# JCBrouwer/maua-style

Measured on AMD Instinct MI355X. Metric: optimizer iterations/sec at 1024x1024 VGG-19, higher is better.
Workload: dtype f32 (fp16x3 split-precision MFMA, fp32 accumulate)

## Files before the change

### include/maua_hip.h

```cpp
#ifndef MAUA_HIP_H
#define MAUA_HIP_H

#include <stddef.h>
#include <stdint.h>

#ifdef __cplusplus
extern "C" {
#endif

typedef void* maua_stream_t;

#define MAUA_OK 0
#define MAUA_E_INVAL (-1)
#define MAUA_E_UNSUPPORTED (-2)
#define MAUA_E_WORKSPACE (-3)

int maua_abi_version(void);
const char* maua_last_error(void);


int maua_conv_pack_filters(const float* w_oihw, float* wf, float* wb, int cout, int cin, int kh, int kw,
                           maua_stream_t stream);

size_t maua_conv_workspace_bytes(int n, int cin, int h, int w, int cout, int kh, int kw, int stride, int pad);
// ... 3 lines not shown

int maua_conv2d_bwd_data(const float* gy, const float* out_mask, const float* wb, const float* w_oihw,
                         const float* in_relu_mask, float* gx, int n, int cin, int h, int w, int cout, int kh, int kw,
                         int stride, int pad, int accumulate, void* workspace, size_t workspace_bytes, maua_stream_t stream);

size_t maua_conv_x6_bank_bytes(int cout_produced, int cin_consumed);
int maua_conv_pack_filters_x6(const float* w_oihw, void* bank_fwd, void* bank_bwd, int cout, int cin, maua_stream_t stream);
size_t maua_conv_x6_workspace_bytes(int n, int cin, int h, int w, int cout, int pad);
int maua_conv3x3_x6(const float* x, const void* bank, const float* bias, const float* out_relu_mask, float* y, int n,
                    int cin, int h, int w, int cout, int pad, int relu, int accumulate, void* workspace,
                    size_t workspace_bytes, maua_stream_t stream);

int maua_conv_image_supported(int n, int cin, int h, int w, int cout, int pad);
size_t maua_conv_image_bank_bytes(int cout, int cin);
int maua_conv_pack_filters_image(const float* w_oihw, const float* bias, void* bank, int cout, int cin, maua_stream_t stream);
int maua_conv3x3_image(const float* x, const void* bank, float* y, int n, int cin, int h, int w, int cout, int pad, int relu,
                       maua_stream_t stream);
int maua_conv_image_gram_slabs(int h, int w, int pad);
int maua_conv3x3_image_gram(const float* x, const void* bank, float* y, float* gram_slabs, int cin, int h, int w, int pad, maua_stream_t stream);

size_t maua_conv_x3_bank_bytes(int cout_produced, int cin_consumed);
int maua_conv_pack_filters_x3(const float* w_oihw, void* bank_fwd, void* bank_bwd, int cout, int cin, float w_scale,
                              maua_stream_t stream);
size_t maua_conv_x3_workspace_bytes(int n, int cin, int h, int w, int cout, int pad);
int maua_conv3x3_x3(const float* x, const void* bank, float w_scale, const float* bias, const float* out_relu_mask, float* y,
                    int n, int cin, int h, int w, int cout, int pad, int relu, int accumulate, void* workspace,
                    size_t workspace_bytes, maua_stream_t stream);

size_t maua_conv_x3w_bank_bytes(int cout_produced, int cin_consumed);
int maua_conv_pack_filters_x3w(const float* w_oihw, void* bank_fwd, void* bank_bwd, int cout, int cin, float w_scale,
                               maua_stream_t stream);
int maua_conv_x3w_supported(int cin, int h, int w, int pad);
size_t maua_conv_x3w_workspace_bytes(int n, int cin, int h, int w, int cout, int pad);
int maua_conv3x3_x3w(const float* x, const void* bank, float w_scale, const float* bias, const float* out_relu_mask, float* y,
                     int n, int cin, int h, int w, int cout, int pad, int relu, int accumulate, void* workspace,
                     size_t workspace_bytes, maua_stream_t stream);

int maua_conv_x3w_split(int n, int cin, int h, int w, int cout, int pad);
int maua_conv3x3_x3w_relu_pool(const float* x, const void* bank, float w_scale, const float* bias, float* pooled,
                               unsigned char* codes, int n, int cin, int h, int w, int cout, int pad, void* workspace,
                               size_t workspace_bytes, maua_stream_t stream);

size_t maua_conv_x3w_dmat_bank_bytes(int c);
int maua_conv_pack_dmat_x3w(const float* dmat, int c, void* bank, float* inv_scale_out, maua_stream_t stream);
int maua_conv_pack_dmat_x3w_batch(int count, const float* const* dmats, const int* cs, void* const* banks, float* const* inv_scales_out,
                                  maua_stream_t stream);
int maua_conv3x3_x3w_gram(const float* x, const void* bank, float w_scale, const float* feature_map, const void* dmat_bank,
                          const float* dmat_inv_scale, float* y, int n, int cin, int h, int w, int cout, int pad, int accumulate,
                          void* workspace, size_t workspace_bytes, maua_stream_t stream);

int maua_conv3x3_x3w_unpool(const float* pooled_x, const unsigned char* codes, int honour_relu_bit, const void* bank, float w_scale,
                            const float* out_relu_mask, const void* dmat_bank, const float* dmat_inv_scale, float* y, int n, int cin,
                            int h, int w, int cout, int pad, void* workspace, size_t workspace_bytes, maua_stream_t stream);

size_t maua_conv_x3q_bank_bytes(int cout_produced, int cin_consumed);
int maua_conv_pack_filters_x3q(const float* w_oihw, void* bank_fwd, void* bank_bwd, int cout, int cin, float w_scale,
                               maua_stream_t stream);
int maua_conv_x3q_supported(int cin, int h, int w, int pad);
size_t maua_conv_x3q_workspace_bytes(int n, int cin, int h, int w, int cout, int pad);
int maua_conv_x3q_split(int n, int cin, int h, int w, int cout, int pad);
int maua_conv_x3q_preferred(int n, int cin, int h, int w, int cout, int pad);
int maua_conv3x3_x3q(const float* x, const void* bank, float w_scale, const float* bias, const float* out_relu_mask, float* y,
                     int n, int cin, int h, int w, int cout, int pad, int relu, int accumulate, void* workspace,
                     size_t workspace_bytes, maua_stream_t stream);
int maua_conv3x3_x3q_relu_pool(const float* x, const void* bank, float w_scale, const float* bias, float* pooled, unsigned char* codes,
                               int n, int cin, int h, int w, int cout, int pad, void* workspace, size_t workspace_bytes,
                               maua_stream_t stream);
int maua_conv3x3_x3q_unpool(const float* pooled_x, const unsigned char* codes, int honour_relu_bit, const void* bank, float w_scale,
                            const float* out_relu_mask, float* y, int n, int cin, int h, int w, int cout, int pad, void* workspace,
                            size_t workspace_bytes, maua_stream_t stream);

int maua_conv_x3p_supported(int cin, int h, int w, int cout, int pad);
int maua_conv_x3p_split(int n, int cin, int h, int w, int cout, int pad);
size_t maua_conv_x3p_workspace_bytes(int n, int cin, int h, int w, int cout, int pad);
int maua_conv_x3p_preferred(int n, int cin, int h, int w, int cout, int pad);
int maua_conv_x3p_set_max_groups(int groups);
int maua_conv3x3_x3p(const float* x, const unsigned char* in_codes, int honour_relu_bit, const void* bank, float w_scale, const float* bias,
                     const float* out_relu_mask, const void* dmat_bank, const float* dmat_inv_scale, float* y, unsigned char* pool_codes,
                     int n, int cin, int h, int w, int cout, int pad, int relu, void* workspace, size_t workspace_bytes, maua_stream_t stream);

size_t maua_conv_kxk_x3_bank_bytes(int cout_produced, int cin_consumed, int ks);
int maua_conv_pack_filters_kxk_x3(const float* w_oihw, void* bank_fwd, void* bank_bwd, int cout, int cin, int ks, float w_scale,
                                  maua_stream_t stream);
size_t maua_conv_kxk_x3_workspace_bytes(int n, int cin, int h, int w, int cout, int ks, int pad);
int maua_conv_kxk_x3(const float* x, const void* bank, float w_scale, const float* bias, const float* out_relu_mask, float* y,
                     int n, int cin, int h, int w, int cout, int ks, int pad, int relu, int accumulate, void* workspace,
                     size_t workspace_bytes, maua_stream_t stream);

size_t maua_conv1x1_x3_workspace_bytes(int n, int cin, int64_t hw, int cout);
int maua_conv1x1_x3(const float* x, const float* x_channel_shift, const float* w_rowmajor, const float* bias,
                    const float* out_relu_mask, float* y, int n, int cin, int64_t hw, int cout, int relu, int accumulate,
                    void* workspace, size_t workspace_bytes, maua_stream_t stream);

int maua_relu_fwd(float* x_inplace, int64_t count, maua_stream_t stream);
int maua_relu_bwd(const float* gy, const float* y, float* gx, int64_t count, maua_stream_t stream);

int maua_pool_out_size(int in, int k, int stride, int ceil_mode);
int maua_pool2d_fwd(const float* x, float* y, int n, int c, int h, int w, int k, int stride, int ceil_mode, int mode,
                    maua_stream_t stream);
int maua_pool2d_bwd(const float* gy, const float* x, float* gx, int n, int c, int h, int w, int k, int stride,
                    int ceil_mode, int mode, int relu_mask_by_x, maua_stream_t stream);

int maua_pool2x2_codes_supported(int n, int c, int h, int w);
int maua_pool2x2_fwd_codes(const float* x, float* y, unsigned char* codes, int n, int c, int h, int w, maua_stream_t stream);
int maua_pool2x2_bwd_codes(const float* gy, const unsigned char* codes, float* gx, int n, int c, int h, int w, int relu_mask,
                           maua_stream_t stream);

size_t maua_gram_workspace_bytes(int c, int64_t hw);
int maua_gram_block(int c, int64_t hw);
int maua_gram_fwd(const float* f, float* gram, float* row_mean_out, int c, int64_t hw, float scale, int center,
                  void* workspace, size_t workspace_bytes, maua_stream_t stream);

size_t maua_reduce_workspace_bytes(int64_t count);
int maua_mse_fwd_bwd(const float* x, const float* target, float* grad, int64_t count, float loss_scale, float grad_scale,
                     int accumulate, int mask_grad_by_x, float* loss_out, void* workspace, size_t workspace_bytes,
                     maua_stream_t stream);
int maua_mse_weighted_fwd_bwd(const float* x, const float* weights, const float* target, float* grad, int64_t planes,
                              int64_t plane, int weight_planes, float loss_scale, float grad_scale, int accumulate,
                              float* loss_out, void* workspace, size_t workspace_bytes, maua_stream_t stream);

int maua_gram_bwd(const float* d_sym, const float* f, const float* row_mean, const float* relu_mask, float* gf, int c,
                  int64_t hw, int accumulate, void* workspace, size_t workspace_bytes, maua_stream_t stream);

int maua_tv_fwd_bwd(const float* x, float* grad, int n, int c, int h, int w, float strength, int accumulate,
                    float* loss_out, void* workspace, size_t workspace_bytes, maua_stream_t stream);

size_t maua_loss_ledger_bytes(int frames, int slots);
int maua_mse_fwd_bwd_ledger(const float* x, const float* target, float* grad, int64_t count, float loss_scale, float grad_scale,
                            int accumulate, int mask_grad_by_x, double* ledger, int slot, maua_stream_t stream);
int maua_tv_fwd_bwd_ledger(const float* x, float* grad, int n, int c, int h, int w, float strength, int accumulate,
                           double* ledger, int slot, maua_stream_t stream);
int maua_gram_mse_ledger_supported(int c);
int maua_gram_fwd_mse_ledger(const float* f, float* gram, float* row_mean_out, int c, int64_t hw, float scale, int center,
                             const float* target, float* dmat, float loss_scale, float grad_scale, double* ledger, int slot,
                             void* workspace, size_t workspace_bytes, maua_stream_t stream);
int maua_gram_partial(const float* f, float* row_mean_out, int c, int64_t hw, int center, void* workspace, size_t workspace_bytes,
                      maua_stream_t stream);
int maua_gram_partial_batch(int count, const float* const* fs, float* const* means, const int* cs, const int64_t* hws,
                            void* const* workspaces, const size_t* workspace_bytes, const int* slab_counts, maua_stream_t stream);
int maua_gram_row_means(const float* f, float* row_mean_out, int c, int64_t hw, void* workspace, size_t workspace_bytes, maua_stream_t stream);
int maua_gram_finish_mse_batch(int count, const void* const* workspaces, float* const* grams, const float* const* targets,
                               float* const* dmats, const int* cs, const int64_t* hws, const float* scales, const float* loss_scales,
                               const float* grad_scales, double* const* ledgers, const int* slots, const int* slab_counts,
                               maua_stream_t stream);
int maua_loss_ledger_sum(double* ledger, int frames, int slots, float* losses, float* totals, maua_stream_t stream);
int maua_loss_ledger_sum_f64(double* ledger, int frames, int slots, float* losses, float* totals, double* losses_f64,
                             maua_stream_t stream);

int maua_fill(float* x, int64_t count, float value, maua_stream_t stream);
size_t maua_conv_few_mfma_bank_bytes(void);
int maua_conv_pack_filters_few_mfma(const float* w_oihw, void* bank, int cout, int cin, maua_stream_t stream);
int maua_conv_few_mfma_supported(int n, int cin, int h, int w, int cout, int pad);
int maua_conv3x3_few_mfma(const float* gy, const void* bank, float* gx, int n, int cin, int h, int w, int cout, int tile, maua_stream_t stream);

int maua_space_to_depth(const float* in, float* out, int n, int c_in, int r, int h, int w, int qh, int qw, maua_stream_t stream);
int maua_depth_to_space(const float* in, float* out, int n, int c_out, int r, int qh, int qw, int h, int w, int accumulate, maua_stream_t stream);
int maua_axpy(float* y, const float* x, float alpha, int64_t count, maua_stream_t stream);
int maua_sum_small(const float* in, int count, float* out, maua_stream_t stream);

int maua_adam_step(float* x, const float* grad, float* exp_avg, float* exp_avg_sq, int64_t count, int step, float lr,
                   float beta1, float beta2, float eps, maua_stream_t stream);

size_t maua_channel_stats_workspace_bytes(int h, int w);
int maua_channel_stats(const float* x_bchw, const float* noise_bwhc, float noise_amp, int frames, int slot, int h, int w,
                       double* stats9, void* workspace, size_t workspace_bytes, maua_stream_t stream);
int maua_color_match_solve(const double* stats_target, int frames, int64_t pixels_target, const double* stats_source,
                           int64_t pixels_source, float eps, float* coef16, maua_stream_t stream);
int maua_color_match_apply(const float* x_bchw, const float* noise_bwhc, float noise_amp, const float* coef16, const float* all_coef,
                           int n_coef, float weight, int accumulate, int frames, int slot, int h, int w, float* out_bchw,
                           maua_stream_t stream);
int maua_resize_bilinear(const float* x, float* y, int planes, int h, int w, int oh, int ow, float scale_h, float scale_w,
                         maua_stream_t stream);
int maua_deprocess_u8(const float* x_bgr_chw, unsigned char* out_rgb_hwc, int h, int w, float mean_b, float mean_g, float mean_r,
                      maua_stream_t stream);

int maua_set_tuning(const char* name, double value);
double maua_get_tuning(const char* name, double dflt);

void maua_set_split_batch_hint(int frames);
int maua_get_split_batch_hint(void);

int maua_conv_arm_workspace(void* workspace, void* counters, size_t counter_bytes, int zero, maua_stream_t stream);

size_t maua_lbfgs_state_bytes(int64_t count, int history);
int maua_lbfgs_init(void* state, size_t state_bytes, int64_t count, int history, maua_stream_t stream);
int maua_lbfgs_iterate(void* state, float* x, const float* grad, const float* loss, int64_t count, int history, float lr,
                       float tolerance_change, float tolerance_grad, maua_stream_t stream);
int maua_lbfgs_status(const void* state, int64_t count, int history, float* out5, maua_stream_t stream);

int maua_flow_levels(int h, int w, int max_levels);
int maua_flow_grey_u8(const uint8_t* rgb, float* out, int h, int w, maua_stream_t stream);
int maua_flow_pyr_down(const float* in, float* out, int h, int w, maua_stream_t stream);
int maua_flow_warp_prep(const float* i0, const float* i1, const float* u, float* fields, int h, int w, maua_stream_t stream);
int maua_flow_tvl1_step(const float* fields, const float* state_in, float* state_out, int h, int w, maua_stream_t stream);
int maua_flow_tvl1_blocked(const float* fields, const float* state_in, float* state_out, int h, int w, int k, maua_stream_t stream);
int maua_flow_median5(const float* in, float* out, int h, int w, int planes, maua_stream_t stream);
int maua_flow_upsample(const float* in, int ch, int cw, float* out, int h, int w, int planes, float scale, maua_stream_t stream);
size_t maua_flow_consistency_workspace_bytes(int h, int w);
int maua_flow_consistency(const float* flow1, const float* flow2, uint8_t* out, int h, int w, void* workspace, size_t workspace_bytes,
                          maua_stream_t stream);
size_t maua_flow_tvl1_workspace_bytes(int h, int w, int levels);
int maua_flow_tvl1(const uint8_t* rgb1, const uint8_t* rgb2, float* flow, int h, int w, int levels, int warps, int iters, int block_k,
                   void* workspace, size_t workspace_bytes, maua_stream_t stream);

int maua_nca_supported(int n, int chn, int hidden, int h, int w);
int64_t maua_nca_param_count(int chn, int hidden);
int maua_nca_step(const float* x, float* out, const float* params, int n, int chn, int hidden, int h, int w, float rate,
                  const float* rate_map, const float* mask, uint64_t seed, int64_t step, maua_stream_t stream);
size_t maua_nca_bwd_workspace_bytes(int n, int chn, int hidden, int h, int w);
int maua_nca_step_bwd(const float* x, const float* g, float* dx, const float* params, int n, int chn, int hidden, int h, int w,
                      float rate, const float* rate_map, const float* mask, uint64_t seed, int64_t step, int first, void* workspace,
                      size_t workspace_bytes, maua_stream_t stream);
int maua_nca_grad_finish(float* grad, int n, int chn, int hidden, int h, int w, const void* workspace, size_t workspace_bytes,
                         int normalize, maua_stream_t stream);

#ifdef __cplusplus
}
#endif
#endif
```

### maua-style_amd/csrc/conv_api.hip

```cpp
#include <cstdlib>
#include <cstring>

#include "common.hpp"

using namespace maua;

namespace maua {
static thread_local int g_split_batch_hint = 1;
int split_batch_hint() { return g_split_batch_hint; }
static thread_local const void* g_armed_ws = nullptr;
static thread_local unsigned* g_armed_counters = nullptr;
unsigned* armed_counters(const void* workspace) { return workspace && workspace == g_armed_ws ? g_armed_counters : nullptr; }
}

namespace maua {
static const char* const g_tuning_names[] = {"conv_few_out", "few_out_ks4_below", "x3w_ks", "x3w_stagger", "x3q_ks", "x3q_min_fill", "x3q_min_chunks",
                                             "x3p_ks", "x3p_groups", "x3p_min_fill", "x3p_min_items", "x6_persist", "gram_x3", "gram_bwd_x3",
                                             "gram_t128", "gram_t128_min_hw", "p1_order", "lbfgs_vec", "lbfgs_tri", "finish_in_launch_max_ks", "x3p_order", "cot_inner"};
constexpr int kTunings = sizeof(g_tuning_names) / sizeof(g_tuning_names[0]);
static double g_tuning_values[kTunings];
static bool g_tuning_set[kTunings];
static int tuning_index(const char* name) {
    for (int i = 0; i < kTunings; ++i)
        if (name && strcmp(name, g_tuning_names[i]) == 0) return i;
    return -1;
}
double tuning(const char* name, double dflt) {
    const int i = tuning_index(name);
    return i >= 0 && g_tuning_set[i] ? g_tuning_values[i] : dflt;
}
}

static inline bool mfma_geometry(int kh, int kw, int stride) {
    return stride == 1 && kh == kw && (kh == 1 || kh == 3 || kh == 5);
}
static int conv_route(const ConvArgs& a, int ks, int n, hipStream_t stream) {
    const bool few_out = tuning("conv_few_out", 1) != 0;
    if (ks == 3 && a.Cout <= 4 && a.Cin >= 16 && few_out) return conv3x3_few_out(a, n, stream);
    return conv_mfma_dispatch(a, ks, n, stream);
}

extern "C" {

int maua_set_tuning(const char* name, double value) {
    const int i = maua::tuning_index(name);
    MAUA_REQUIRE(i >= 0, MAUA_E_INVAL, "set_tuning: unknown constant %s", name ? name : "(null)");
    maua::g_tuning_values[i] = value;
    maua::g_tuning_set[i] = true;
    return MAUA_OK;
}
double maua_get_tuning(const char* name, double dflt) { return maua::tuning(name, dflt); }

int maua_conv_arm_workspace(void* workspace, void* counters, size_t counter_bytes, int zero, maua_stream_t stream) {
    if (!workspace || !counters) {
        maua::g_armed_ws = nullptr;
        maua::g_armed_counters = nullptr;
        return MAUA_OK;
    }
    MAUA_REQUIRE(counter_bytes >= (size_t)maua::ARRIVE_COUNTERS * 4 && ((size_t)counters & 15) == 0, MAUA_E_INVAL,
                 "conv_arm_workspace: needs %d bytes of 16-byte aligned counters", maua::ARRIVE_COUNTERS * 4);
    const hipError_t rc = zero ? hipMemsetAsync(counters, 0, (size_t)maua::ARRIVE_COUNTERS * 4, (hipStream_t)stream) : hipSuccess;
    if (rc != hipSuccess) {
        set_error("conv_arm_workspace: hipMemsetAsync: %s", hipGetErrorString(rc));
        return (int)rc;
    }
    maua::g_armed_ws = workspace;
    maua::g_armed_counters = (unsigned*)counters;
    return MAUA_OK;
}

void maua_set_split_batch_hint(int frames) { maua::g_split_batch_hint = frames > 0 ? frames : 1; }
int maua_get_split_batch_hint(void) { return maua::g_split_batch_hint; }

size_t maua_conv_workspace_bytes(int n, int cin, int h, int w, int cout, int kh, int kw, int stride, int pad) {
    if (!conv_dims_ok(n, cin, h, w, cout, pad) || kh <= 0 || kw <= 0 || kh > 64 || kw > 64 || stride <= 0 || stride > 64) return 0;
    if (!mfma_geometry(kh, kw, stride) || h + 2 * pad < kh || w + 2 * pad < kw) return 0;
    ConvArgs a{};
    a.Cin = cin;
    a.Cout = cout;
    a.OH = h + 2 * pad - kh + 1;
    a.OW = w + 2 * pad - kw + 1;
    if (kh == 3 && cout <= 4 && cin >= 16) return 0;
    const int ks = conv_mfma2_choose_split(a, kh, n);
    return ks > 1 ? (size_t)n * ks * cout * a.OH * a.OW * sizeof(float) : 0;
}

int maua_conv2d_fwd(const float* x, const float* in_mask, const float* wf, const float* bias, float* y, int n, int cin,
                    int h, int w, int cout, int kh, int kw, int stride, int pad, int relu, int accumulate, void* workspace,
                    size_t workspace_bytes, maua_stream_t stream) {
    MAUA_REQUIRE(x && wf && y, MAUA_E_INVAL, "conv2d_fwd: null pointer");
    MAUA_REQUIRE(conv_dims_ok(n, cin, h, w, cout, pad) && kh > 0 && kw > 0 && kh <= 64 && kw <= 64 && stride > 0 && stride <= 64, MAUA_E_INVAL,
                 "conv2d_fwd: bad dims n=%d cin=%d cout=%d h=%d w=%d k=%dx%d s=%d p=%d", n, cin, cout, h, w, kh, kw, stride,
                 pad);
    const int oh = (h + 2 * pad - kh) / stride + 1, ow = (w + 2 * pad - kw) / stride + 1;
    MAUA_REQUIRE(h + 2 * pad >= kh && w + 2 * pad >= kw, MAUA_E_UNSUPPORTED, "conv2d_fwd: input %dx%d smaller than filter", h,
                 w);
    MAUA_REQUIRE((int64_t)h * w < (1ll << 31) && (int64_t)oh * ow < (1ll << 31), MAUA_E_UNSUPPORTED,
                 "conv2d_fwd: plane too large");
    if (mfma_geometry(kh, kw, stride)) {
        ConvArgs a{};
        a.x = x;
        a.mask = in_mask;
        a.w = wf;
        a.bias = bias;
        a.y = y;
        a.Cin = cin;
        a.H = h;
        a.W = w;
        a.Cout = cout;
        a.OH = oh;
        a.OW = ow;
        a.pad = pad;
        a.relu = relu;
        a.accumulate = accumulate;
        a.ws = (workspace && workspace_bytes >= maua_conv_workspace_bytes(n, cin, h, w, cout, kh, kw, stride, pad))
                   ? (float*)workspace : nullptr;
        return conv_route(a, kh, n, (hipStream_t)stream);
    }
    return conv_direct_fwd(x, in_mask, wf, bias, y, n, cin, h, w, cout, oh, ow, kh, kw, stride, pad, relu, accumulate,
                           (hipStream_t)stream);
}

int maua_conv2d_bwd_data(const float* gy, const float* out_mask, const float* wb, const float* w_oihw,
                         const float* in_relu_mask, float* gx, int n, int cin, int h, int w, int cout, int kh, int kw,
                         int stride, int pad, int accumulate, void* workspace, size_t workspace_bytes, maua_stream_t stream) {
    MAUA_REQUIRE(gy && gx && (wb || w_oihw), MAUA_E_INVAL, "conv2d_bwd_data: null pointer");
    MAUA_REQUIRE(conv_dims_ok(n, cin, h, w, cout, pad) && kh > 0 && kw > 0 && kh <= 64 && kw <= 64 && stride > 0 && stride <= 64, MAUA_E_INVAL,
                 "conv2d_bwd_data: bad dims");
    const int oh = (h + 2 * pad - kh) / stride + 1, ow = (w + 2 * pad - kw) / stride + 1;
    MAUA_REQUIRE(h + 2 * pad >= kh && w + 2 * pad >= kw, MAUA_E_UNSUPPORTED, "conv2d_bwd_data: input smaller than filter");
    if (mfma_geometry(kh, kw, stride) && wb) {
        ConvArgs a{};
        a.x = gy;
        a.mask = out_mask;
        a.w = wb;
        a.bias = nullptr;
        a.omask = in_relu_mask;
        a.y = gx;
        a.Cin = cout;
        a.H = oh;
        a.W = ow;
        a.Cout = cin;
        a.OH = h;
        a.OW = w;
        a.pad = kh - 1 - pad;
        a.relu = 0;
        a.accumulate = accumulate;
        MAUA_REQUIRE(a.pad >= 0, MAUA_E_UNSUPPORTED, "conv2d_bwd_data: pad %d > k-1", pad);
        a.ws = (workspace && workspace_bytes >= maua_conv_workspace_bytes(n, cout, oh, ow, cin, kh, kw, 1, a.pad))
                   ? (float*)workspace : nullptr;
        return conv_route(a, kh, n, (hipStream_t)stream);
    }
    MAUA_REQUIRE(w_oihw, MAUA_E_INVAL, "conv2d_bwd_data: the direct path needs the OIHW weights");
    return conv_direct_bwd(gy, out_mask, w_oihw, in_relu_mask, gx, n, cin, h, w, cout, oh, ow, kh, kw, stride, pad, accumulate,
                           (hipStream_t)stream);
}

}
```

### maua-style_amd/csrc/conv_few_mfma.hip

```cpp
#include <hip/hip_runtime.h>

#include "common.hpp"

namespace maua {

typedef __attribute__((ext_vector_type(8))) __bf16 fm_bf16x8;
typedef __attribute__((ext_vector_type(16))) float fm_f32x16;
typedef __attribute__((ext_vector_type(4))) unsigned int fm_u32x4;
typedef float fm_f32x2 __attribute__((ext_vector_type(2)));
typedef __bf16 fm_bf16x2 __attribute__((ext_vector_type(2)));

__device__ __forceinline__ unsigned short fm_bf16_bits(float x) { return __builtin_bit_cast(unsigned short, (__bf16)x); }
__device__ __forceinline__ float fm_bf16_value(unsigned short u) { return __builtin_bit_cast(float, (unsigned)u << 16); }
__device__ __forceinline__ unsigned fm_cvt_pk(float a, float b) {
    const fm_f32x2 v = {a, b};
    return __builtin_bit_cast(unsigned, __builtin_convertvector(v, fm_bf16x2));
}

constexpr int FM_K = 64;
constexpr int FM_STEPS = FM_K / 16;
constexpr int FM_TC = 64, FM_OC = 62;
constexpr int FM_BANK_BYTES = FM_STEPS * 3 * 64 * 16;

__global__ void pack_few_mfma_kernel(const float* __restrict__ w, unsigned short* __restrict__ bank, int co) {
    const int total = FM_STEPS * 64 * 8;
    for (int e = blockIdx.x * blockDim.x + threadIdx.x; e < total; e += gridDim.x * blockDim.x) {
        const int i = e % 8, lane = (e / 8) % 64, step = e / 512;
        const int m = lane & 31, k = 16 * step + 8 * (lane >> 5) + i;
        float v = 0.f;
        if (m < 9 * co) {
            const int tap = m / co, c = m - tap * co;
            v = w[((int64_t)k * co + c) * 9 + tap];
        }
        const unsigned short h = fm_bf16_bits(v);
        const float r1 = v - fm_bf16_value(h);
        const unsigned short md = fm_bf16_bits(r1);
        const unsigned short l = fm_bf16_bits(r1 - fm_bf16_value(md));
        const unsigned short parts[3] = {h, md, l};
        for (int part = 0; part < 3; ++part) bank[(((int64_t)step * 3 + part) * 64 + lane) * 8 + i] = parts[part];
    }
}

struct FewMfmaArgs {
    const float* gy;
    const unsigned char* bank;
    float* gx;
    int H, W, co;
    int tiles_x, tiles, per_xcd;
};

template <int ROWS>
__global__ void __launch_bounds__(256, 2) conv_few_mfma_kernel(FewMfmaArgs p) {
    extern __shared__ float T[];
    constexpr int TR = ROWS + 2, TPL = TR * FM_TC, NBLK = TR * 2;
    const int tid = threadIdx.x, lane = tid & 63, wave = tid >> 6, nl = lane & 31, kg = lane >> 5;
    const int tile = (int)(blockIdx.x & 7) * p.per_xcd + (int)(blockIdx.x >> 3);
    if (tile >= p.tiles) return;
    const int ty = tile / p.tiles_x;
    const int x0 = (tile - ty * p.tiles_x) * FM_OC, y0 = ty * ROWS, img = blockIdx.z;
    const int64_t plane = (int64_t)p.H * p.W;
    fm_bf16x8 a[FM_STEPS][3];
#pragma unroll
    for (int step = 0; step < FM_STEPS; ++step)
#pragma unroll
        for (int part = 0; part < 3; ++part)
            a[step][part] = *reinterpret_cast<const fm_bf16x8*>(p.bank + (((step * 3 + part) * 64) + lane) * 16);
    const __amdgpu_buffer_rsrc_t rs = __builtin_amdgcn_make_buffer_rsrc(const_cast<float*>(p.gy) + (int64_t)img * FM_K * plane, 0,
                                                                        (unsigned)(FM_K * plane * 4), 0x00020000);
    auto request = [&](float (&v)[FM_STEPS][8], int b) {
        const int tr = b >> 1, Y = y0 - 1 + tr, X = x0 - 1 + 32 * (b & 1) + nl;
        const bool ok = Y >= 0 && Y < p.H && X >= 0 && X < p.W;
        const unsigned voff = ok ? (unsigned)(((int64_t)kg * 8 * plane + (int64_t)Y * p.W + X) * 4) : 0x80000000u;
#pragma unroll
        for (int step = 0; step < FM_STEPS; ++step)
#pragma unroll
            for (int i = 0; i < 8; ++i)
                v[step][i] = __builtin_bit_cast(float, __builtin_amdgcn_raw_buffer_load_b32(rs, voff, (unsigned)((16 * step + i) * plane * 4), 0));
    };
    float v[FM_STEPS][8], vn[FM_STEPS][8];
    if (wave < NBLK) request(v, wave);
    for (int b = wave; b < NBLK; b += 4) {
        if (b + 4 < NBLK) request(vn, b + 4);
        fm_f32x16 acc;
#pragma unroll
        for (int r = 0; r < 16; ++r) acc[r] = 0.f;
#pragma unroll
        for (int step = 0; step < FM_STEPS; ++step) {
            fm_u32x4 bp[3];
#pragma unroll
            for (int q = 0; q < 4; ++q) {
                const float u0 = v[step][2 * q], u1 = v[step][2 * q + 1];
                const unsigned h = fm_cvt_pk(u0, u1);
                const float r0 = u0 - __builtin_bit_cast(float, h << 16), r1 = u1 - __builtin_bit_cast(float, h & 0xffff0000u);
                const unsigned m = fm_cvt_pk(r0, r1);
                const unsigned l = fm_cvt_pk(r0 - __builtin_bit_cast(float, m << 16), r1 - __builtin_bit_cast(float, m & 0xffff0000u));
                bp[0][q] = h;
                bp[1][q] = m;
                bp[2][q] = l;
            }
            const fm_bf16x8 b0v = __builtin_bit_cast(fm_bf16x8, bp[0]), b1v = __builtin_bit_cast(fm_bf16x8, bp[1]),
                            b2v = __builtin_bit_cast(fm_bf16x8, bp[2]);
            acc = __builtin_amdgcn_mfma_f32_32x32x16_bf16(a[step][2], b0v, acc, 0, 0, 0);
            acc = __builtin_amdgcn_mfma_f32_32x32x16_bf16(a[step][1], b1v, acc, 0, 0, 0);
            acc = __builtin_amdgcn_mfma_f32_32x32x16_bf16(a[step][0], b2v, acc, 0, 0, 0);
            acc = __builtin_amdgcn_mfma_f32_32x32x16_bf16(a[step][1], b0v, acc, 0, 0, 0);
            acc = __builtin_amdgcn_mfma_f32_32x32x16_bf16(a[step][0], b1v, acc, 0, 0, 0);
            acc = __builtin_amdgcn_mfma_f32_32x32x16_bf16(a[step][0], b0v, acc, 0, 0, 0);
        }
        float* dst = T + (b >> 1) * FM_TC + 32 * (b & 1) + nl;
#pragma unroll
        for (int r = 0; r < 16; ++r) {
            const int m = (r & 3) + 8 * (r >> 2) + 4 * kg;
            if (m < 9 * p.co) dst[m * TPL] = acc[r];
        }
#pragma unroll
        for (int step = 0; step < FM_STEPS; ++step)
#pragma unroll
            for (int i = 0; i < 8; ++i) v[step][i] = vn[step][i];
    }
    __syncthreads();
    const int co = p.co;
    for (int idx = tid; idx < ROWS * FM_OC; idx += 256) {
        const int i = idx / FM_OC, j = idx - i * FM_OC;
        const int Y = y0 + i, X = x0 + j;
        if (Y >= p.H || X >= p.W) continue;
        const float* t0 = T + (i + 2) * FM_TC + j + 2;
        for (int c = 0; c < co; ++c) {
            float s = 0.f;
#pragma unroll
            for (int ky = 0; ky < 3; ++ky)
#pragma unroll
                for (int kx = 0; kx < 3; ++kx) s += t0[((ky * 3 + kx) * co + c) * TPL - ky * FM_TC - kx];
            p.gx[((int64_t)img * co + c) * plane + (int64_t)Y * p.W + X] = s;
        }
    }
}

}

using namespace maua;

extern "C" {

size_t maua_conv_few_mfma_bank_bytes(void) { return FM_BANK_BYTES; }

int maua_conv_pack_filters_few_mfma(const float* w_oihw, void* bank, int cout, int cin, maua_stream_t stream) {
    MAUA_REQUIRE(w_oihw && bank, MAUA_E_INVAL, "conv_pack_filters_few_mfma: null pointer");
    MAUA_REQUIRE(cout == FM_K && cin >= 1 && cin <= 3, MAUA_E_UNSUPPORTED, "conv_pack_filters_few_mfma: a 3x3 layer with %d filters over 1-3 channels (got %d over %d)", FM_K, cout, cin);
    hipLaunchKernelGGL(pack_few_mfma_kernel, dim3(8), dim3(256), 0, (hipStream_t)stream, w_oihw, (unsigned short*)bank, cin);
    return check_launch("pack_few_mfma_kernel");
}

int maua_conv_few_mfma_supported(int n, int cin, int h, int w, int cout, int pad) {
    return conv_dims_ok(n, cin, h, w, cout, pad) && cout == FM_K && cin >= 1 && cin <= 3 && pad == 1 && n <= 65535 && (int64_t)FM_K * h * w * 4 < (1ll << 31) &&
           (h + 3) / 4 <= 65535;
}

int maua_conv3x3_few_mfma(const float* gy, const void* bank, float* gx, int n, int cin, int h, int w, int cout, int tile, maua_stream_t stream) {
    MAUA_REQUIRE(gy && bank && gx, MAUA_E_INVAL, "conv3x3_few_mfma: null pointer");
    MAUA_REQUIRE(maua_conv_few_mfma_supported(n, cin, h, w, cout, 1), MAUA_E_UNSUPPORTED, "conv3x3_few_mfma: unsupported geometry");
    MAUA_REQUIRE(tile >= 0 && tile <= 3, MAUA_E_INVAL, "conv3x3_few_mfma: tile code 0 - 3");
    if (tile == 0) tile = (int64_t)h * w < 1000000 ? 1 : 2;
    FewMfmaArgs p{gy, (const unsigned char*)bank, gx, h, w, cin, 0, 0, 0};
    static unsigned long long attr[4] = {0, 0, 0, 0};
    const int rows = tile == 1 ? 4 : tile == 2 ? 8 : 14;
    const int lds = 27 * (rows + 2) * FM_TC * 4;
    p.tiles_x = (w + FM_OC - 1) / FM_OC;
    p.tiles = p.tiles_x * ((h + rows - 1) / rows);
    p.per_xcd = (p.tiles + 7) / 8;
    const dim3 grid((unsigned)(8 * p.per_xcd), 1, (unsigned)n);
    if (rows == 4) {
        (void)opt_in_dynamic_lds(reinterpret_cast<const void*>(conv_few_mfma_kernel<4>), lds, &attr[1]);
        hipLaunchKernelGGL(conv_few_mfma_kernel<4>, grid, dim3(256), lds, (hipStream_t)stream, p);
    } else if (rows == 8) {
        (void)opt_in_dynamic_lds(reinterpret_cast<const void*>(conv_few_mfma_kernel<8>), lds, &attr[2]);
        hipLaunchKernelGGL(conv_few_mfma_kernel<8>, grid, dim3(256), lds, (hipStream_t)stream, p);
    } else {
        (void)opt_in_dynamic_lds(reinterpret_cast<const void*>(conv_few_mfma_kernel<14>), lds, &attr[3]);
        hipLaunchKernelGGL(conv_few_mfma_kernel<14>, grid, dim3(256), lds, (hipStream_t)stream, p);
    }
    return check_launch("conv_few_mfma_kernel");
}

}
```

### maua-style_amd/csrc/conv_img.hip

```cpp
#include <hip/hip_runtime.h>

#include "common.hpp"

namespace maua {

typedef __attribute__((ext_vector_type(8))) __bf16 ci_bf16x8;
typedef __attribute__((ext_vector_type(16))) float ci_f32x16;
typedef __attribute__((ext_vector_type(4))) unsigned int ci_u32x4;
typedef float ci_f32x2 __attribute__((ext_vector_type(2)));
typedef __bf16 ci_bf16x2 __attribute__((ext_vector_type(2)));

__device__ __forceinline__ unsigned short ci_bf16_bits(float x) { return __builtin_bit_cast(unsigned short, (__bf16)x); }
__device__ __forceinline__ float ci_bf16_value(unsigned short u) { return __builtin_bit_cast(float, (unsigned)u << 16); }
__device__ __forceinline__ unsigned ci_cvt_pk(float a, float b) {
    const ci_f32x2 v = {a, b};
    return __builtin_bit_cast(unsigned, __builtin_convertvector(v, ci_bf16x2));
}

constexpr int CI_KPAD = 32;
#ifndef CI_OCC
#define CI_OCC 2
#endif
constexpr int CI_TILE_BYTES = 2 * 2 * 3 * 64 * 16;

__global__ void pack_image_kernel(const float* __restrict__ w, const float* __restrict__ bias, unsigned short* __restrict__ bank, int cout,
                                  int cin) {
    const int ntile = (cout + 63) / 64;
    const int64_t total = (int64_t)ntile * 2 * 2 * 64 * 8;
    for (int64_t e = (int64_t)blockIdx.x * blockDim.x + threadIdx.x; e < total; e += (int64_t)gridDim.x * blockDim.x) {
        int64_t r = e;
        const int i = (int)(r % 8);
        r /= 8;
        const int lane = (int)(r % 64);
        r /= 64;
        const int step = (int)(r % 2);
        r /= 2;
        const int blk = (int)(r % 2);
        const int tile = (int)(r / 2);
        const int co = tile * 64 + blk * 32 + (lane & 31), k = 16 * step + 8 * (lane >> 5) + i;
        float v = 0.f;
        if (co < cout && k < 9 * cin) v = w[(int64_t)co * cin * 9 + k];
        if (co < cout && k == 9 * cin && bias) v = bias[co];
        const unsigned short h = ci_bf16_bits(v);
        const float r1 = v - ci_bf16_value(h);
        const unsigned short m = ci_bf16_bits(r1);
        const unsigned short l = ci_bf16_bits(r1 - ci_bf16_value(m));
        const unsigned short parts[3] = {h, m, l};
        for (int part = 0; part < 3; ++part)
            bank[(((((int64_t)tile * 2 + blk) * 2 + step) * 3 + part) * 64 + lane) * 8 + i] = parts[part];
    }
}

struct ImgArgs {
    const float* x;
    const unsigned char* bank;
    float* y;
    float* gram_slabs;
    int n, cin, H, W, cout, OH, OW, pad, relu;
    int blocks_x;
    int64_t blocks;
};

template <bool GRAM>
__global__ void __launch_bounds__(256, CI_OCC) conv_image_kernel(ImgArgs p) {
    const int lane = threadIdx.x & 63;
    const int nl = lane & 31, kg = lane >> 5;
    const int tile = blockIdx.y;
    ci_bf16x8 a[2][2][3];
    {
        const unsigned char* src = p.bank + (int64_t)tile * CI_TILE_BYTES + lane * 16;
#pragma unroll
        for (int blk = 0; blk < 2; ++blk)
#pragma unroll
            for (int step = 0; step < 2; ++step)
#pragma unroll
                for (int part = 0; part < 3; ++part)
                    a[blk][step][part] = *reinterpret_cast<const ci_bf16x8*>(src + (((blk * 2 + step) * 3 + part) * 64) * 16);
    }
    const int64_t plane = (int64_t)p.H * p.W;
    const int kmax = 9 * p.cin;
    int rel[2][8];
    unsigned ones = 0;
#pragma unroll
    for (int step = 0; step < 2; ++step)
#pragma unroll
        for (int i = 0; i < 8; ++i) {
            int k = 16 * step + 8 * kg + i;
            if (k == kmax) ones |= 1u << (8 * step + i);
            k = k < kmax ? k : 0;
            const int ci = k / 9, ky = (k - 9 * ci) / 3, kx = k - 9 * ci - 3 * ky;
            rel[step][i] = (int)(ci * plane) + (ky - p.pad) * p.W + (kx - p.pad);
        }
    const int64_t out_plane = (int64_t)p.OH * p.OW;
    const int nw = (int)gridDim.x * 4;
    const int wid = __builtin_amdgcn_readfirstlane((int)blockIdx.x * 4 + (int)(threadIdx.x >> 6));
    const int per = (int)((p.blocks + nw - 1) / nw);
    const int b0 = wid * per, b1 = (int)(p.blocks < (int64_t)b0 + per ? p.blocks : (int64_t)b0 + per);
    ci_f32x16 gsum[3];
    if constexpr (GRAM) {
#pragma unroll
        for (int q = 0; q < 3; ++q)
#pragma unroll
            for (int r = 0; r < 16; ++r) gsum[q][r] = 0.f;
    }
    if (!GRAM && b0 >= b1) return;
    int bx = b0 < b1 ? b0 % p.blocks_x : 0, oy = b0 < b1 ? (b0 / p.blocks_x) % p.OH : 0, img = b0 < b1 ? (b0 / p.blocks_x) / p.OH : 0;
    auto gather = [&](float (&v)[2][8], int gi, int gy, int gb) {
        const int ox = gb * 32 + nl;
        const float* __restrict__ xin = p.x + (int64_t)gi * p.cin * plane;
        const int centre = gy * p.W + ox;
        const bool interior = gy - p.pad >= 0 && gy - p.pad + 2 < p.H && gb * 32 - p.pad >= 0 && gb * 32 + 31 - p.pad + 2 < p.W;
        if (interior) {
#pragma unroll
            for (int step = 0; step < 2; ++step)
#pragma unroll
                for (int i = 0; i < 8; ++i) v[step][i] = xin[centre + rel[step][i]];
        } else {
#pragma unroll
            for (int step = 0; step < 2; ++step)
#pragma unroll
                for (int i = 0; i < 8; ++i) {
                    int k = 16 * step + 8 * kg + i;
                    k = k < kmax ? k : 0;
                    const int t9 = k % 9;
                    const int iy = gy + t9 / 3 - p.pad, ix = ox + t9 % 3 - p.pad;
                    const bool ok = iy >= 0 && iy < p.H && ix >= 0 && ix < p.W;
                    v[step][i] = ok ? xin[centre + rel[step][i]] : 0.f;
                }
        }
    };
    float v[2][8], vn[2][8];
    if (b0 < b1) gather(v, img, oy, bx);
    for (int b = b0; b < b1; ++b) {
        bx = __builtin_amdgcn_readfirstlane(bx);
        oy = __builtin_amdgcn_readfirstlane(oy);
        img = __builtin_amdgcn_readfirstlane(img);
        int nbx = bx + 1, noy = oy, nimg = img;
        if (nbx == p.blocks_x) {
            nbx = 0;
            if (++noy == p.OH) {
                noy = 0;
                ++nimg;
            }
        }
        if (b + 1 < b1) gather(vn, nimg, noy, nbx);
#pragma unroll
        for (int step = 0; step < 2; ++step)
#pragma unroll
            for (int i = 0; i < 8; ++i) v[step][i] = (ones >> (8 * step + i)) & 1u ? 1.f : v[step][i];
        ci_u32x4 bp[2][3];
#pragma unroll
        for (int step = 0; step < 2; ++step)
#pragma unroll
            for (int q = 0; q < 4; ++q) {
                const float x0 = v[step][2 * q], x1 = v[step][2 * q + 1];
                const unsigned h = ci_cvt_pk(x0, x1);
                const float r0 = x0 - __builtin_bit_cast(float, h << 16), r1 = x1 - __builtin_bit_cast(float, h & 0xffff0000u);
                const unsigned m = ci_cvt_pk(r0, r1);
                const unsigned l = ci_cvt_pk(r0 - __builtin_bit_cast(float, m << 16), r1 - __builtin_bit_cast(float, m & 0xffff0000u));
                bp[step][0][q] = h;
                bp[step][1][q] = m;
                bp[step][2][q] = l;
            }
        ci_f32x16 acc[2];
#pragma unroll
        for (int blk = 0; blk < 2; ++blk)
#pragma unroll
            for (int r = 0; r < 16; ++r) acc[blk][r] = 0.f;
#pragma unroll
        for (int step = 0; step < 2; ++step) {
            const ci_bf16x8 b0v = __builtin_bit_cast(ci_bf16x8, bp[step][0]), b1v = __builtin_bit_cast(ci_bf16x8, bp[step][1]),
                            b2v = __builtin_bit_cast(ci_bf16x8, bp[step][2]);
#define CI_PAIR(AP, BV)                                                                                         \
    acc[0] = __builtin_amdgcn_mfma_f32_32x32x16_bf16(a[0][step][AP], BV, acc[0], 0, 0, 0);                       \
    acc[1] = __builtin_amdgcn_mfma_f32_32x32x16_bf16(a[1][step][AP], BV, acc[1], 0, 0, 0);
            CI_PAIR(2, b0v) CI_PAIR(1, b1v) CI_PAIR(0, b2v) CI_PAIR(1, b0v) CI_PAIR(0, b1v) CI_PAIR(0, b0v)
#undef CI_PAIR
        }
        const int ox = bx * 32 + nl;
        const int tile_ch = min(64, p.cout - tile * 64);
        const __amdgpu_buffer_rsrc_t rs = __builtin_amdgcn_make_buffer_rsrc(p.y + ((int64_t)img * p.cout + tile * 64) * out_plane, 0,
                                                                            (unsigned)(tile_ch * out_plane * 4), 0x00020000);
        const unsigned voff = ox < p.OW ? (unsigned)((4 * kg * out_plane + (int64_t)oy * p.OW + ox) * 4) : 0x80000000u;
#pragma unroll
        for (int blk = 0; blk < 2; ++blk)
#pragma unroll
            for (int r = 0; r < 16; ++r) {
                const int cr = blk * 32 + (r & 3) + 8 * (r >> 2);
                float o = acc[blk][r];
                if (p.relu) o = o > 0.f ? o : 0.f;
                __builtin_amdgcn_raw_buffer_store_b32(__builtin_bit_cast(unsigned, o), rs, voff, (int)(cr * out_plane * 4), 0);
            }
        if constexpr (GRAM) {
            ci_f32x16 xt[2];
#pragma unroll
            for (int blk = 0; blk < 2; ++blk)
#pragma unroll
                for (int r = 0; r < 16; ++r) xt[blk][r] = 0.f;
#pragma unroll
            for (int step = 0; step < 2; ++step) {
                const ci_bf16x8 b0v = __builtin_bit_cast(ci_bf16x8, bp[step][0]), b1v = __builtin_bit_cast(ci_bf16x8, bp[step][1]),
                                b2v = __builtin_bit_cast(ci_bf16x8, bp[step][2]);
#define CI_PAIR_T(AP, BV)                                                                                       \
    xt[0] = __builtin_amdgcn_mfma_f32_32x32x16_bf16(BV, a[0][step][AP], xt[0], 0, 0, 0);                         \
    xt[1] = __builtin_amdgcn_mfma_f32_32x32x16_bf16(BV, a[1][step][AP], xt[1], 0, 0, 0);
                CI_PAIR_T(2, b0v) CI_PAIR_T(1, b1v) CI_PAIR_T(0, b2v) CI_PAIR_T(1, b0v) CI_PAIR_T(0, b1v) CI_PAIR_T(0, b0v)
#undef CI_PAIR_T
            }
            ci_u32x4 fr[2][2][3];
            const int px0 = bx * 32 + 4 * kg;
#pragma unroll
            for (int blk = 0; blk < 2; ++blk)
#pragma unroll
                for (int sK = 0; sK < 2; ++sK)
#pragma unroll
                    for (int q = 0; q < 4; ++q) {
                        const int r0i = 8 * sK + 2 * q, r1i = r0i + 1;
                        float x0 = xt[blk][r0i], x1 = xt[blk][r1i];
                        x0 = (x0 > 0.f && px0 + (r0i & 3) + 8 * (r0i >> 2) < p.OW) ? x0 : 0.f;
                        x1 = (x1 > 0.f && px0 + (r1i & 3) + 8 * (r1i >> 2) < p.OW) ? x1 : 0.f;
                        const unsigned h = ci_cvt_pk(x0, x1);
                        const float e0 = x0 - __builtin_bit_cast(float, h << 16), e1 = x1 - __builtin_bit_cast(float, h & 0xffff0000u);
                        const unsigned m = ci_cvt_pk(e0, e1);
                        const unsigned l = ci_cvt_pk(e0 - __builtin_bit_cast(float, m << 16), e1 - __builtin_bit_cast(float, m & 0xffff0000u));
                        fr[blk][sK][0][q] = h;
                        fr[blk][sK][1][q] = m;
                        fr[blk][sK][2][q] = l;
                    }
#pragma unroll
            for (int sK = 0; sK < 2; ++sK) {
#define CI_G(PA, PB)                                                                                                                        \
    gsum[0] = __builtin_amdgcn_mfma_f32_32x32x16_bf16(__builtin_bit_cast(ci_bf16x8, fr[0][sK][PA]), __builtin_bit_cast(ci_bf16x8, fr[0][sK][PB]), gsum[0], 0, 0, 0); \
    gsum[1] = __builtin_amdgcn_mfma_f32_32x32x16_bf16(__builtin_bit_cast(ci_bf16x8, fr[0][sK][PA]), __builtin_bit_cast(ci_bf16x8, fr[1][sK][PB]), gsum[1], 0, 0, 0); \
    gsum[2] = __builtin_amdgcn_mfma_f32_32x32x16_bf16(__builtin_bit_cast(ci_bf16x8, fr[1][sK][PA]), __builtin_bit_cast(ci_bf16x8, fr[1][sK][PB]), gsum[2], 0, 0, 0);
                CI_G(2, 0) CI_G(1, 1) CI_G(0, 2) CI_G(1, 0) CI_G(0, 1) CI_G(0, 0)
#undef CI_G
            }
        }
#pragma unroll
        for (int step = 0; step < 2; ++step)
#pragma unroll
            for (int i = 0; i < 8; ++i) v[step][i] = vn[step][i];
        bx = nbx;
        oy = noy;
        img = nimg;
    }
    if constexpr (GRAM) {
        __shared__ float red[3][3][16][64];
        const int wave = threadIdx.x >> 6;
        if (wave > 0) {
#pragma unroll
            for (int q = 0; q < 3; ++q)
#pragma unroll
                for (int r = 0; r < 16; ++r) red[wave - 1][q][r][lane] = gsum[q][r];
        }
        __syncthreads();
        if (wave > 0) return;
        float* __restrict__ slab = p.gram_slabs + (int64_t)blockIdx.x * 64 * 64;
#pragma unroll
        for (int q = 0; q < 3; ++q) {
            const int bi = q == 2 ? 1 : 0, bj = q == 0 ? 0 : 1;
#pragma unroll
            for (int r = 0; r < 16; ++r) {
                float g = gsum[q][r];
#pragma unroll
                for (int w = 0; w < 3; ++w) g += red[w][q][r][lane];
                slab[(bi * 32 + (r & 3) + 8 * (r >> 2) + 4 * kg) * 64 + bj * 32 + nl] = g;
            }
        }
    }
}

}

using namespace maua;

extern "C" {

size_t maua_conv_image_bank_bytes(int cout, int cin) {
    if (cout <= 0 || cin <= 0 || cin > 3 || cout > (1 << 16)) return 0;
    return (size_t)((cout + 63) / 64) * CI_TILE_BYTES;
}

int maua_conv_pack_filters_image(const float* w_oihw, const float* bias, void* bank, int cout, int cin, maua_stream_t stream) {
    MAUA_REQUIRE(w_oihw && bank && cout > 0 && cout <= (1 << 16) && cin > 0 && cin <= 3, MAUA_E_INVAL,
                 "conv_pack_filters_image: needs 1-3 input channels");
    hipLaunchKernelGGL(pack_image_kernel, dim3(32), dim3(256), 0, (hipStream_t)stream, w_oihw, bias, (unsigned short*)bank, cout, cin);
    return check_launch("pack_image_kernel");
}

static bool conv_image_fits(int64_t n, int64_t cin, int64_t h, int64_t w, int64_t pad) {
    const int64_t oh = h + 2 * pad - 2, ow = w + 2 * pad - 2;
    return cin * h * w < (1ll << 31) && n * oh * ((ow + 31) / 32) < (1ll << 31) && 64 * oh * ow < (1ll << 30);
}

static int conv_image_fill(ImgArgs& p, const float* x, const void* bank, float* y, int n, int cin, int h, int w, int cout, int pad, int relu) {
    MAUA_REQUIRE(x && bank && y, MAUA_E_INVAL, "conv3x3_image: null pointer");
    MAUA_REQUIRE(conv_dims_ok(n, cin, h, w, cout, pad) && pad <= 2 && cin <= 3, MAUA_E_INVAL, "conv3x3_image: bad dims (1-3 input channels)");
    MAUA_REQUIRE(h + 2 * pad >= 3 && w + 2 * pad >= 3, MAUA_E_UNSUPPORTED, "conv3x3_image: input smaller than the filter");
    MAUA_REQUIRE(conv_image_fits(n, cin, h, w, pad), MAUA_E_UNSUPPORTED, "conv3x3_image: plane too large (maua_conv_image_supported)");
    p.x = x;
    p.bank = (const unsigned char*)bank;
    p.y = y;
    p.n = n;
    p.cin = cin;
    p.H = h;
    p.W = w;
    p.cout = cout;
    p.OH = h + 2 * pad - 2;
    p.OW = w + 2 * pad - 2;
    p.pad = pad;
    p.relu = relu;
    p.blocks_x = (p.OW + 31) / 32;
    p.blocks = (int64_t)n * p.OH * p.blocks_x;
    return MAUA_OK;
}
static unsigned conv_image_grid(int64_t blocks) {
    const int64_t want = (blocks + 3) / 4;
    return (unsigned)(want < 256 * CI_OCC ? (want > 0 ? want : 1) : 256 * CI_OCC);
}

int maua_conv3x3_image(const float* x, const void* bank, float* y, int n, int cin, int h, int w, int cout, int pad, int relu,
                       maua_stream_t stream) {
    ImgArgs p{};
    const int rc = conv_image_fill(p, x, bank, y, n, cin, h, w, cout, pad, relu);
    if (rc) return rc;
    hipLaunchKernelGGL(conv_image_kernel<false>, dim3(conv_image_grid(p.blocks), (unsigned)((cout + 63) / 64)), dim3(256), 0, (hipStream_t)stream, p);
    return check_launch("conv_image_kernel");
}

int maua_conv_image_supported(int n, int cin, int h, int w, int cout, int pad) {
    return conv_dims_ok(n, cin, h, w, cout, pad) && pad <= 2 && cin <= 3 && h + 2 * pad >= 3 && w + 2 * pad >= 3 && conv_image_fits(n, cin, h, w, pad);
}

int maua_conv_image_gram_slabs(int h, int w, int pad) {
    if (h <= 0 || w <= 0 || pad < 0 || pad > 2 || h + 2 * pad < 3 || w + 2 * pad < 3 || !conv_image_fits(1, 3, h, w, pad)) return 0;
    const int64_t oh = h + 2 * pad - 2, ow = w + 2 * pad - 2;
    return (int)conv_image_grid(oh * ((ow + 31) / 32));
}

int maua_conv3x3_image_gram(const float* x, const void* bank, float* y, float* gram_slabs, int cin, int h, int w, int pad, maua_stream_t stream) {
    MAUA_REQUIRE(gram_slabs, MAUA_E_INVAL, "conv3x3_image_gram: null slabs");
    ImgArgs p{};
    const int rc = conv_image_fill(p, x, bank, y, 1, cin, h, w, 64, pad, 1);
    if (rc) return rc;
    p.gram_slabs = gram_slabs;
    hipLaunchKernelGGL(conv_image_kernel<true>, dim3(conv_image_grid(p.blocks), 1), dim3(256), 0, (hipStream_t)stream, p);
    return check_launch("conv_image_kernel");
}

}
```

### maua-style_amd/engine.py

```python
import contextlib
import os

import torch

import hip
import loss as loss_mod
import models as models_mod
import plan


class UnsupportedNet(RuntimeError):
    """The module sequence contains something the fused plan does not cover (callers fall back to running the
    modules one by one, which still executes on the GPU through the same kernels)."""


def _scale_grad_coeff(incoming, strength):
    g = float(incoming)
    return g / (abs(g) + 1e-8) * strength * strength


class _Step:
    __slots__ = ("kind", "mod", "relu", "src", "dst", "slot", "k", "stride", "pad", "ceil", "mode")

    def __init__(self, kind, mod=None):
# ... 123 lines not shown
                if len(users) == 1 and users[0].kind == "pool" and id(users[0]) in self.pool_codes and \
                        self._x6_ok(s, s.mod.out_channels) and models_mod.conv3x3_fwd_is_x3w(s.mod, *shapes[s.src][2:]) and \
                        s.mod.out_channels % 8 == 0 and (plan.on("fuse_pool_split") or models_mod.conv3x3_fwd_family(
                            s.mod, B, shapes[s.src][2], shapes[s.src][3])[1] == 1):
                    self.fused_pool[id(s)] = users[0]
        self.pooled_by_conv = {id(v) for v in self.fused_pool.values()}
        for s in self.steps:
            if id(s) in self.fused_pool:
                self.act[s.dst] = torch.empty(shapes[s.dst], device="meta")
        self.fused_unpool, self.pool_groups = {}, set()
        if self.x6_bwd:
            for s in self.steps:
                if s.kind != "conv" or not s.relu or s.k != 3 or s.stride != 1 or s.pad != 1:
                    continue
                users = [t for t in self.steps if t.src == s.dst and t is not s]
                if len(users) == 1 and users[0].kind == "pool" and id(users[0]) in self.pool_codes and \
                        self._x6_ok(s, s.mod.in_channels) and models_mod.conv3x3_bwd_is_x3w(s.mod, *shapes[s.dst][2:]):
                    self.pool_groups.add(id(s))
                    if plan.on("fuse_unpool"):
                        self.fused_unpool[id(s)] = users[0]
                        self.gbuf[s.dst] = torch.empty(shapes[s.dst], device="meta")
        self.unpooled_by_conv = {id(v) for v in self.fused_unpool.values()}
        self.fused_gram = {}
        max_c = plan.get_int("fuse_gram_max_c")
        if (B == 1 or self.independent) and self.x6_bwd and max_c > 0:
            relu_out = {s.dst for s in self.steps if s.kind == "conv" and s.relu}
            for s in self.steps:
                if s.kind != "conv" or s.k != 3 or s.stride != 1 or s.pad != 1 or s.src not in relu_out:
                    continue
                on_src = [t for t in self.steps if t.kind in ("style", "content") and t.src == s.src]
                c, h, w = shapes[s.src][1:]
                if len(on_src) == 1 and on_src[0].kind == "style" and not on_src[0].mod.use_covariance and c % 16 == 0 and \
                        c <= max_c and self._x6_ok(s, s.mod.in_channels) and models_mod.conv3x3_bwd_is_x3w(s.mod, *shapes[s.dst][2:]):
                    bank = hip.conv_x3w_dmat_bank(c, dev, B)
                    if bank is not None:
                        self.fused_gram[id(s)] = (on_src[0], bank[0], bank[1])
        self.fused_style = {id(v[0]): v for v in self.fused_gram.values()}
        self.image_gram = {}
        if B == 1 and self.batch_hint == 1 and self.ledger is not None and self.x6_fwd and plan.on("image_gram") and \
                plan.on("gram_x3") and models_mod._image_kernel_enabled():
            for s in self.steps:
                if s.kind != "conv" or not s.relu or s.k != 3 or s.stride != 1 or s.mod.in_channels > 3 or s.mod.out_channels != 64 or \
                        not self._x6_ok(s, 64):
                    continue
                on_dst = [t for t in self.steps if t.kind == "style" and t.src == s.dst]
                if len(on_dst) == 1 and not on_dst[0].mod.use_covariance and hip.gram_mse_ledger_supported(64):
                    h, w = shapes[s.src][2:]
                    slabs = hip.conv_image_gram_slabs(h, w, s.pad)
                    if 0 < slabs * 64 * 64 * 4 <= hip.gram_workspace_bytes(64, shapes[s.dst][2] * shapes[s.dst][3]):
                        self.image_gram[id(s)] = (on_dst[0], slabs)
        self.gram, self.dmat, self.mean = {}, {}, {}
        self.gram_d, self.dmat_d, self.mean_d = {}, {}, {}
        ws = hip.reduce_workspace_bytes(max(t.numel() for t in self.gbuf.values()))
        for s in self.steps:
            if s.kind == "style":
                c = shapes[s.src][1]
                hw = shapes[s.src][2] * shapes[s.src][3]
                self.gram[id(s)] = torch.empty(B, c, c, device=dev) if B > 1 else torch.empty(c, c, device=dev)
                self.dmat[id(s)] = torch.empty(B, c, c, device=dev) if B > 1 else torch.empty(c, c, device=dev)
                self.mean[id(s)] = (torch.empty(B, c, device=dev) if B > 1 else torch.empty(c, device=dev)) \
                    if s.mod.use_covariance else None
                ws = max(ws, hip.gram_workspace_bytes(c, hw), 4 * c + 256)
                if B > 1 and not self.independent:
                    self.gram_d[id(s)] = torch.empty(B * c, B * c, device=dev)
                    self.dmat_d[id(s)] = torch.empty(B * c, B * c, device=dev)
                    self.mean_d[id(s)] = torch.empty(B * c, device=dev) if s.mod.use_covariance else None
                    ws = max(ws, hip.gram_workspace_bytes(B * c, hw), 4 * B * c + 256)
        for s in self.steps:
            if s.kind == "conv" and s.stride == 1:
                n, cin, h, w = shapes[s.src]
                _, cout, oh, ow = shapes[s.dst]
                ws = max(ws, hip.conv_workspace_bytes(n, cin, h, w, cout, s.k, 1, s.pad),
                         hip.conv_workspace_bytes(n, cout, oh, ow, cin, s.k, 1, s.k - 1 - s.pad))
                if s.k == 5:
                    ws = max(ws, hip.conv_kxk_x3_workspace_bytes(n, cin, h, w, cout, 5, s.pad),
                             hip.conv_kxk_x3_workspace_bytes(n, cout, oh, ow, cin, 5, 4 - s.pad))
                if s.k == 1 and s.pad == 0:
                    ws = max(ws, hip.conv1x1_x3_workspace_bytes(n, cin, h * w, cout), hip.conv1x1_x3_workspace_bytes(n, cout, h * w, cin))
                if s.k == 3:
                    ws = max(ws, hip.conv_x6_workspace_bytes(n, cin, h, w, cout, s.pad),
                             hip.conv_x6_workspace_bytes(n, cout, oh, ow, cin, 2 - s.pad),
                             hip.conv_x3_workspace_bytes(n, cin, h, w, cout, s.pad),
                             hip.conv_x3_workspace_bytes(n, cout, oh, ow, cin, 2 - s.pad),
                             hip.conv_x3w_workspace_bytes(n, cin, h, w, cout, s.pad),
                             hip.conv_x3w_workspace_bytes(n, cout, oh, ow, cin, 2 - s.pad),
                             hip.conv_x3q_workspace_bytes(n, cin, h, w, cout, s.pad),
                             hip.conv_x3q_workspace_bytes(n, cout, oh, ow, cin, 2 - s.pad),
                             hip.conv_x3p_workspace_bytes(n, cin, h, w, cout, s.pad),
                             hip.conv_x3p_workspace_bytes(n, cout, oh, ow, cin, 2 - s.pad))
        self.strided_sites, self.strided_fwd_sites = {}, {}
        for s in self.steps:
            if s.kind == "conv" and s.stride > 1 and self.x6_fwd and models_mod.conv_strided_fwd_is_3x3(s.mod, *shapes[s.src][2:]):
                n, cin, h, w = shapes[s.src]
                qh, qw = shapes[s.dst][2] + 2, shapes[s.dst][3] + 2
                self.strided_fwd_sites[id(s)] = torch.empty(n, s.stride * s.stride * cin, qh, qw, device=dev)
                ws = max(ws, hip.conv_x3w_workspace_bytes(n, s.stride * s.stride * cin, qh, qw, s.mod.out_channels, 0))
        for s in self.steps:
            if s.kind == "conv" and s.stride > 1 and self.x6_bwd and models_mod.conv_strided_bwd_is_3x3(s.mod, *shapes[s.dst][2:]):
                n, cin, _, _ = shapes[s.src]
                _, cout, oh, ow = shapes[s.dst]
                self.strided_sites[id(s)] = torch.empty(n, s.stride * s.stride * cin, oh + 2, ow + 2, device=dev)
                ws = max(ws, hip.conv_x3w_workspace_bytes(n, cout, oh, ow, s.stride * s.stride * cin, 2))
        self.ws = torch.empty(ws, dtype=torch.uint8, device=dev)
        self.x_static = torch.empty(self.shape, device=dev)
        if plan.get("debug_poison") == "1":
            for t in list(self.act.values()) + list(self.gbuf.values()) + list(self.gram.values()) + list(self.dmat.values()) + \
                    list(self.gram_d.values()) + list(self.dmat_d.values()):
                if t is not None and not t.is_meta:
                    t.fill_(float("nan"))
            self.ws[:self.ws.numel() // 4 * 4].view(torch.float32)[:] = float("nan")
        self.ws_counters = torch.empty(hip.ARRIVAL_COUNTER_BYTES, dtype=torch.uint8, device=dev) if plan.on("finish_in_launch") and ws > 0 else None
        self.ws_armed_epoch = None
        self.side, self.side_ws, self.ev_main, self.ev_side = [], [], None, []
        aside = plan.get("style_stream")
        self.style_aside = B == 1 and self.ledger is not None and \
            (aside == "1" or (aside == "auto" and x.shape[2] * x.shape[3] >= 1536 * 1536))
        if (B > 1 and self.independent and plan.get_int("side_streams") > 0) or self.style_aside:
            ns = min(B, plan.get_int("side_streams")) if B > 1 else 1
            small = hip.reduce_workspace_bytes(max(t.numel() for t in self.gbuf.values()) // B)
            for s in self.steps:
                if s.kind == "style":
                    c, hw = shapes[s.src][1], shapes[s.src][2] * shapes[s.src][3]
                    small = max(small, hip.gram_workspace_bytes(c, hw), 4 * c + 256)
            self.side = [torch.cuda.Stream(device=dev) for _ in range(ns)]
            self.side_ws = [torch.empty(small, dtype=torch.uint8, device=dev) for _ in range(ns)]
            self.ev_main = torch.cuda.Event()
            self.ev_side = [torch.cuda.Event() for _ in range(ns)]

    def _style_terms(self, s, B):
        m = s.mod
        st, vsf = m.strength, m.video_style_factor
        static = (st / B, _scale_grad_coeff(st / B, st) if m.normalize else st / B)
        dynamic = None
        if vsf > 0:
            if m.video_target.nelement() == 0:
                raise RuntimeError(f"{m.name}: dynamic style target not captured")
            if m.video_target.shape[0] == B * m.target.shape[0]:
                dynamic = (vsf * st / B, _scale_grad_coeff(vsf * st / B, st) if m.normalize else vsf * st / B)
        return static, dynamic

    def _coefficients(self, s):
        m = s.mod
        st = m.strength
        if s.kind == "content":
            return st, (_scale_grad_coeff(st, st) if m.normalize else st)
        vsf = m.video_style_factor
        dyn = vsf > 0
        lw = st + (vsf * st if dyn else 0.0)
        if m.normalize:
            gw = _scale_grad_coeff(st, st) + (_scale_grad_coeff(vsf * st, st) if dyn else 0.0)
        else:
            gw = lw
        return lw, gw

    def _active(self, s, shapes_src):
        m = s.mod
        if s.kind == "tv":
            return True
        if m.mode != "loss":
            return False
        if s.kind == "content":
            if m.target.nelement() == 0:
                return False
            if tuple(m.target.shape[1:]) != tuple(shapes_src[1:]):
                return False
            if shapes_src[0] > 1 and self.independent:
                if m.weights is not None or m.target.shape[0] != shapes_src[0]:
                    raise UnsupportedNet("independent frames need one unweighted content target per frame")
            elif shapes_src[0] > 1 and (m.weights is not None or m.target.shape[0] != 1):
                raise UnsupportedNet("weighted / multi-frame-target ContentLoss on B > 1 frames runs on the module path")
            if m.weights is not None:
                w = m.weights
                if s.src != 0 or w.dim() != 4 or w.shape[0] != 1 or tuple(w.shape[2:]) != tuple(shapes_src[2:]) \
                        or w.shape[1] not in (1, shapes_src[1]):
                    raise UnsupportedNet("weighted ContentLoss of this shape runs on the module path")
            return True
        if m.target.nelement() == 0:
            raise RuntimeError(f"{m.name}: style target not captured")
        if shapes_src[0] == 1 and m.video_style_factor > 0 and m.video_target.nelement() != 0 \
                and m.video_target.shape != m.target.shape:
            raise UnsupportedNet("dynamic style target of another shape")
        return True

    def _arm(self):
        if self.ws_counters is None:
            hip.conv_arm_workspace(None)
            return
        if self.ws_armed_epoch != (self.ws.data_ptr(), self.ws_counters.data_ptr()):
            hip.conv_arm_workspace(self.ws, self.ws_counters)
            self.ws_armed_epoch = (self.ws.data_ptr(), self.ws_counters.data_ptr())
        else:
            hip.conv_arm_workspace(self.ws, self.ws_counters, zero=False)

    def fork(self):
        if self.side:
            self.ev_main.record()
            for st in self.side:
                st.wait_event(self.ev_main)

    def join(self):
        cur = torch.cuda.current_stream()
        for st, ev in zip(self.side, self.ev_side):
            ev.record(st)
            cur.wait_event(ev)

    def _gram_ws(self, s, c, hw, dev):
        need = hip.gram_workspace_bytes(c, hw)
        t = self._gram_wsp.get(id(s))
        if t is None or t.numel() < need or t.device != dev:
            t = torch.empty(need, dtype=torch.uint8, device=dev)
            self._gram_wsp[id(s)] = t
        return t

    def frame_stream(self, b):
        if not self.side:
            import contextlib
            return contextlib.nullcontext(), self.ws
        k = b % len(self.side)
        return torch.cuda.stream(self.side[k]), self.side_ws[k]

    def _timed(self, tag, flops, nbytes, fn):
        if self.timer is None:
            return fn()
        e0, e1 = torch.cuda.Event(enable_timing=True), torch.cuda.Event(enable_timing=True)
        e0.record()
        out = fn()
        e1.record()
        self.timer.append((tag, flops, nbytes, e0, e1))
        return out

    @staticmethod
    def _conv_work(s, in_shape, out_shape, backward):
        _, cin, h, w = in_shape
        _, cout, oh, ow = out_shape
        flops = 2 * cin * cout * s.k * s.k * oh * ow
        wbytes = (cin * cout * s.k * s.k + cout) * 4
        ib, ob = cin * h * w * 4, cout * oh * ow * 4
        nbytes = (ob + ob + wbytes + ib) if backward else (ib + wbytes + ob)
        return flops, nbytes

    def _image_gram_now(self, s, shape):
        st, _ = self.image_gram[id(s)]
        return self.gram_batch_on and self.gram_partial_batch_on and self._active(st, self.act[s.dst].shape)

    def image_gram_slabs(self, style_step):
        return next(n for st, n in self.image_gram.values() if st is style_step)

    def _x6_ok(self, s, produced_channels):
        return self.use_x6 and s.k == 3 and s.stride == 1 and s.pad <= 2 and produced_channels >= plan.get_int("split_min_produced")

    def _run(self, x):
        hip.set_split_batch_hint(self.batch_hint)
        self._arm()
        a, g = self.act, self.gbuf
        a[0] = x
        hip.fill_(self.slots_all, 0.0)
        forked = False
        batch = []
        emitted = set()
        for s in self.steps:
            if s.kind == "conv":
                fl, nb = self._conv_work(s, a[s.src].shape, a[s.dst].shape, False)
                if id(s) in self.fused_pool:
                    ps = self.fused_pool[id(s)]
                    self._timed("conv3x3_split_fwd", fl, nb, lambda: models_mod.conv3x3_relu_pool(
                        a[s.src], s.mod, a[ps.dst], self.pool_codes[id(ps)], workspace=self.ws))
                elif id(s) in self.image_gram and self._image_gram_now(s, a[s.src].shape):
                    st, _ = self.image_gram[id(s)]
                    gws = self._gram_ws(st, 64, a[s.dst].shape[2] * a[s.dst].shape[3], x.device)
                    models_mod._route("conv_image", a[s.src], s.mod.out_channels, s.pad, False, "27 (channel, tap) pairs as K, bf16x6", relu=True, gram_slabs=True)
                    self._timed("conv3x3_split_fwd", fl, nb, lambda: hip.conv3x3_image_gram(a[s.src], s.mod.bank_image(), s.pad, a[s.dst], gws))
                    emitted.add(id(st))
                elif self.x6_fwd and self._x6_ok(s, s.mod.out_channels):
                    self._timed("conv3x3_split_fwd", fl, nb, lambda: models_mod.conv3x3_mfma(
                        a[s.src], s.mod, False, out=a[s.dst], relu=s.relu, workspace=self.ws))
                elif self.x6_fwd and models_mod.conv1x1_is_mfma(s.mod, False):
                    self._timed("conv_1x1_fwd", fl, nb, lambda: models_mod.conv1x1_mfma(
                        a[s.src], s.mod, False, out=a[s.dst], relu=s.relu, workspace=self.ws))
                elif self.x6_fwd and models_mod.conv5x5_is_mfma(s.mod, False):
                    self._timed("conv_5x5_fwd", fl, nb, lambda: models_mod.conv5x5_mfma(
                        a[s.src], s.mod, False, out=a[s.dst], relu=s.relu, workspace=self.ws))
                elif id(s) in self.strided_fwd_sites:
                    self._timed("conv_other_fwd", fl, nb, lambda: models_mod.conv_strided_fwd_as_3x3(
                        a[s.src], s.mod, a[s.dst], s.relu, self.strided_fwd_sites[id(s)], workspace=self.ws))
                else:
                    wf, _ = s.mod.banks()
                    models_mod._route("conv2d_fwd", a[s.src], s.mod.out_channels, s.pad, False, "direct / fp32 MFMA", relu=s.relu)
                    self._timed("conv_other_fwd", fl, nb, lambda: hip.conv2d_fwd(
                        a[s.src], wf, s.mod.bias_device(), s.k, s.stride, s.pad, s.relu, out=a[s.dst], workspace=self.ws))
            elif s.kind == "relu":
                hip.relu_(a[s.src])
            elif s.kind == "pool":
                if id(s) in self.pooled_by_conv:
                    pass
                elif id(s) in self.pool_codes:
                    hip.pool2x2_fwd_codes(a[s.src], a[s.dst], self.pool_codes[id(s)])
                else:
                    hip.pool2d_fwd(a[s.src], s.k, s.stride, s.ceil, s.mode, out=a[s.dst])
            elif s.kind == "style" and self.independent and a[s.src].shape[0] > 1 and self._active(s, a[s.src].shape):
                f = a[s.src]
                c, n = f.shape[1], f[0].nelement()
                lw, gw = self._coefficients(s)
                fs = self.fused_style.get(id(s))
                self.fork()
                for b in range(f.shape[0]):
                    mean_b = self.mean[id(s)][b] if s.mod.use_covariance else None
# ... 72 lines not shown
                            key = (id(s), l["target"].data_ptr(), l["workspace"].data_ptr(), l["gram"].data_ptr(), l["dmat"].data_ptr(),
                                   l["ledger"].data_ptr(), l["slot"], l["loss_scale"], l["grad_scale"], l["slabs"])
                            fin = self._gram_batches.get(("img", id(s)))
                            if fin is None or fin[0] != key:
                                fin = (key, hip.GramFinishBatch([l]))
                                self._gram_batches[("img", id(s))] = fin
                            fin[1].run_partial()
                            fin[1].run()
                        else:
                            self._timed("gram_fwd", 2 * c * c * (n // c), n * 4 + c * c * 4, lambda: hip.gram_fwd_mse_ledger(
                                f, 1.0 / n, s.mod.use_covariance, self.gram[id(s)], self.mean[id(s)], s.mod.target, self.dmat[id(s)],
                                lw / (c * c), gw * 4.0 / (c * c) / n, self.ledger[0], s.slot, workspace=wsb))
                        if id(s) in self.fused_style:
                            hip.conv_pack_dmat_x3w(self.dmat[id(s)], self.fused_style[id(s)][1][0], self.fused_style[id(s)][2])
                    continue
                self._timed("gram_fwd", 2 * c * c * (n // c), n * 4 + c * c * 4, lambda: hip.gram_fwd(
                    f, 1.0 / n, s.mod.use_covariance, out=self.gram[id(s)], mean_out=self.mean[id(s)], workspace=self.ws))
                hip.mse_fwd_bwd(self.gram[id(s)], s.mod.target, self.dmat[id(s)], lw / (c * c), gw * 4.0 / (c * c) / n,
                                False, self.slots[s.slot:s.slot + 1], workspace=self.ws)
                if id(s) in self.fused_style:
                    hip.conv_pack_dmat_x3w(self.dmat[id(s)], self.fused_style[id(s)][1][0], self.fused_style[id(s)][2])
        if batch:
            for k0 in range(0, len(batch), 8):
                grp = batch[k0:k0 + 8]
                key = tuple((id(l["step"]), l["target"].data_ptr(), l["workspace"].data_ptr(), l["gram"].data_ptr(), l["dmat"].data_ptr(),
                             l["ledger"].data_ptr(), l["slot"], l["loss_scale"], l["grad_scale"],
                             None if l["f"] is None else l["f"].data_ptr(), l["slabs"]) for l in grp)
                later = self.gram_partial_batch_on
                fin = self._gram_batches.get(k0)
                if fin is None or fin[0] != key:
                    fin = (key, hip.GramFinishBatch(grp))
                    self._gram_batches[k0] = fin
                if later:
                    self._timed("gram_fwd", sum(2 * l["c"] * l["c"] * l["hw"] for l in grp), sum(l["c"] * l["hw"] * 4 for l in grp), fin[1].run_partial)
                self._timed("gram_fwd", 0, sum(l["c"] * l["c"] * 8 for l in grp), fin[1].run)
            packs = [(l["dmat"], self.fused_style[id(l["step"])][1][0], self.fused_style[id(l["step"])][2]) for l in batch
                     if id(l["step"]) in self.fused_style]
            if not plan.on("dmat_pack_batch"):
                for d, b, i in packs:
                    hip.conv_pack_dmat_x3w(d, b, i)
                packs = []
            for k0 in range(0, len(packs), 4):
                grp = packs[k0:k0 + 4]
                key = tuple((d.data_ptr(), b.data_ptr(), i.data_ptr()) for d, b, i in grp)
                pk = self._gram_batches.get(("pack", k0))
                if pk is None or pk[0] != key:
                    pk = (key, hip.DmatPackBatch(grp))
                    self._gram_batches[("pack", k0)] = pk
                pk[1].run()
        final_writer = {}
        for s in self.steps:
            if s.kind in ("conv", "pool") or (s.kind in ("style", "content") and self._active(s, a[s.src].shape)):
                final_writer.setdefault(s.src, s)
        relu_acts = {s.dst for s in self.steps if s.kind == "conv" and s.relu}

        def premask(s):
            return final_writer.get(s.src) is s and s.src in relu_acts

        fused_done = set()
        cur = None
        indep = self.independent and x.shape[0] > 1
        if indep or forked:
            self.join()
        for s in reversed(self.steps):
            if indep and s.kind in ("style", "content", "tv"):
                if s.kind != "tv" and not self._active(s, a[s.src].shape):
                    continue
                if id(s) in fused_done:
                    continue
                f = a[s.src]
                acc = cur == s.src
                last_step = s.kind == "tv"
                self.fork()
                for b in range(f.shape[0]):
                    slot = self.slots_all[b, s.slot:s.slot + 1]
                    ctx, wsb = self.frame_stream(b)
                    with ctx:
                        if s.kind == "style":
                            c, n = f.shape[1], f[0].nelement()
                            self._timed("gram_bwd", 2 * c * c * (n // c), n * 4 * 3 + c * c * 4, lambda: hip.gram_bwd(
                                self.dmat[id(s)][b], f[b], self.mean[id(s)][b] if s.mod.use_covariance else None, g[s.src][b],
                                acc, workspace=wsb, relu_mask=f[b] if premask(s) else None))
                        elif s.kind == "content":
                            lw, gw = self._coefficients(s)
                            n = f[0].nelement()
                            if self.ledger is not None:
                                hip.mse_fwd_bwd_ledger(f[b], s.mod.target[b], g[s.src][b], lw / n, gw * 2.0 / n, acc, self.ledger[b],
                                                       s.slot, mask_grad_by_x=premask(s))
                            else:
                                hip.mse_fwd_bwd(f[b], s.mod.target[b], g[s.src][b], lw / n, gw * 2.0 / n, acc, slot, workspace=wsb,
                                                mask_grad_by_x=premask(s))
                        elif self.ledger is not None:
                            hip.tv_fwd_bwd_ledger(f[b:b + 1], g[0][b:b + 1], s.mod.strength, acc, self.ledger[b], s.slot)
                        else:
                            hip.tv_fwd_bwd(f[b:b + 1], g[0][b:b + 1], s.mod.strength, acc, slot, workspace=wsb)
                self.join()
                cur = s.src
            elif s.kind == "style" and a[s.src].shape[0] > 1:
                if self._active(s, a[s.src].shape):
                    f = a[s.src]
                    B, c, n = f.shape[0], f.shape[1], f[0].nelement()
                    _, dynamic = self._style_terms(s, B)
                    acc = cur == s.src
                    cov = s.mod.use_covariance
                    if dynamic is not None:
                        bc = B * c
                        self._timed("gram_bwd", 2 * bc * bc * (n // c), B * n * 4 * 3 + bc * bc * 4, lambda: hip.gram_bwd(
                            self.dmat_d[id(s)], f, self.mean_d[id(s)], g[s.src], acc, workspace=self.ws,
                            relu_mask=f if premask(s) else None))
                    else:
                        for b in range(B):
                            self._timed("gram_bwd", 2 * c * c * (n // c), n * 4 * 3 + c * c * 4, lambda: hip.gram_bwd(
                                self.dmat[id(s)][b], f[b], self.mean[id(s)][b] if cov else None, g[s.src][b], acc,
                                workspace=self.ws, relu_mask=f[b] if premask(s) else None))
                    cur = s.src
            elif s.kind == "content" and a[s.src].shape[0] > 1:
                if self._active(s, a[s.src].shape):
                    x = a[s.src]
                    B, n = x.shape[0], x[0].nelement()
                    st = s.mod.strength
                    lw = st / B
                    gw = _scale_grad_coeff(st / B, st) if s.mod.normalize else st / B
                    slots = self.terms[id(s)]
                    for b in range(B):
                        hip.mse_fwd_bwd(x[b], s.mod.target[0], g[s.src][b], lw / n, gw * 2.0 / n, cur == s.src,
                                        self.slots_all[slots[b]:slots[b] + 1], workspace=self.ws, mask_grad_by_x=premask(s))
                    cur = s.src
            elif s.kind == "style":
                if id(s) in fused_done:
                    continue
                if self._active(s, a[s.src].shape):
                    f = a[s.src]
                    c, n = f.shape[1], f[0].nelement()
                    acc = cur == s.src
                    rm = f if premask(s) else None
                    self._timed("gram_bwd", 2 * c * c * (n // c), n * 4 * 3 + c * c * 4, lambda: hip.gram_bwd(
                        self.dmat[id(s)], f, self.mean[id(s)], g[s.src], acc, workspace=self.ws, relu_mask=rm))
                    cur = s.src
            elif s.kind == "content":
                if self._active(s, a[s.src].shape):
                    lw, gw = self._coefficients(s)
                    n = a[s.src].nelement()
                    if s.mod.weights is not None:
                        hip.mse_weighted_fwd_bwd(a[s.src], s.mod.weights, s.mod.target, g[s.src], lw / n, gw * 2.0 / n,
                                                 cur == s.src, self.slots[s.slot:s.slot + 1], workspace=self.ws)
                    elif self.ledger is not None:
                        hip.mse_fwd_bwd_ledger(a[s.src], s.mod.target, g[s.src], lw / n, gw * 2.0 / n, cur == s.src, self.ledger[0],
                                               s.slot, mask_grad_by_x=premask(s))
                    else:
                        hip.mse_fwd_bwd(a[s.src], s.mod.target, g[s.src], lw / n, gw * 2.0 / n, cur == s.src,
                                        self.slots[s.slot:s.slot + 1], workspace=self.ws, mask_grad_by_x=premask(s))
                    cur = s.src
            elif s.kind == "tv":
                if self.ledger is not None:
                    hip.tv_fwd_bwd_ledger(a[0], g[0], s.mod.strength, cur == 0, self.ledger[0], s.slot)
                else:
                    hip.tv_fwd_bwd(a[0], g[0], s.mod.strength, cur == 0, self.slots[s.slot:s.slot + 1], workspace=self.ws)
                cur = 0
            elif cur is None:
                continue
            elif s.kind == "conv":
                assert cur == s.dst
                fl, nb = self._conv_work(s, a[s.src].shape, a[s.dst].shape, True)
                im = a[s.src] if premask(s) else None
                fg = self.fused_gram.get(id(s))
                with_gram = fg is not None and self._active(fg[0], a[s.src].shape) and premask(fg[0])
                up = self.fused_unpool.get(id(s))
                if up is not None:
                    c, n = a[s.src].shape[1], a[s.src][0].nelement()
                    self._timed("conv3x3_split_bwd", fl + (2 * c * c * (n // c) if with_gram else 0), nb, lambda: models_mod.conv3x3_bwd_from_pooled(
                        g[up.dst], self.pool_codes[id(up)], premask(up), s.mod, g[s.src], out_relu_mask=a[s.src] if with_gram else im,
                        dmat_bank=fg[1] if with_gram else None, dmat_inv_scale=fg[2] if with_gram else None, workspace=self.ws))
                    if with_gram:
                        fused_done.add(id(fg[0]))
                elif with_gram:
                    c, n = a[s.src].shape[1], a[s.src][0].nelement()
                    self._timed("conv3x3_split_bwd", fl + 2 * c * c * (n // c), nb, lambda: models_mod.conv3x3_bwd_with_gram(
                        g[s.dst], s.mod, a[s.src], fg[1], fg[2], out=g[s.src], workspace=self.ws))
                    fused_done.add(id(fg[0]))
                elif self.x6_bwd and self._x6_ok(s, s.mod.in_channels):
                    self._timed("conv3x3_split_bwd", fl, nb, lambda: models_mod.conv3x3_mfma(
                        g[s.dst], s.mod, True, out=g[s.src], out_relu_mask=im, workspace=self.ws, pool_group=id(s) in self.pool_groups))
                elif self.x6_bwd and models_mod.conv1x1_is_mfma(s.mod, True):
                    self._timed("conv_1x1_bwd", fl, nb, lambda: models_mod.conv1x1_mfma(
                        g[s.dst], s.mod, True, out=g[s.src], out_relu_mask=im, workspace=self.ws))
                elif self.x6_bwd and models_mod.conv5x5_is_mfma(s.mod, True):
                    self._timed("conv_5x5_bwd", fl, nb, lambda: models_mod.conv5x5_mfma(
                        g[s.dst], s.mod, True, out=g[s.src], out_relu_mask=im, workspace=self.ws))
                elif im is None and models_mod.conv_few_is_mfma(s.mod, *g[s.dst].shape[0:1], *g[s.dst].shape[2:]):
                    self._timed("conv_other_bwd", fl, nb, lambda: models_mod.conv_few_mfma(g[s.dst], s.mod, g[s.src]))
                elif id(s) in self.strided_sites and im is None:
                    self._timed("conv_other_bwd", fl, nb, lambda: models_mod.conv_strided_bwd_as_3x3(
                        g[s.dst], s.mod, g[s.src], workspace=self.ws, sites=self.strided_sites[id(s)]))
                else:
                    _, wb = s.mod.banks()
                    models_mod._route("conv3x3_few_out" if s.k == 3 and s.stride == 1 and s.mod.in_channels <= 4 and s.mod.out_channels >= 16 else "conv2d_bwd_data",
                                      g[s.dst], s.mod.in_channels, s.k - 1 - s.pad, True, "direct / fp32 MFMA", mask=im is not None)
                    self._timed("conv_other_bwd", fl, nb, lambda: hip.conv2d_bwd_data(
                        g[s.dst], None, wb, s.mod.weight.detach(), a[s.src].shape, s.k, s.stride, s.pad, out=g[s.src],
                        in_relu_mask=im, workspace=self.ws))
                cur = s.src
            elif s.kind == "relu":
                hip.relu_bwd(g[s.src], a[s.src], out=g[s.src])
            elif s.kind == "pool":
                assert cur == s.dst
                if id(s) in self.unpooled_by_conv:
                    pass
                elif id(s) in self.pool_codes:
                    hip.pool2x2_bwd_codes(g[s.dst], self.pool_codes[id(s)], g[s.src], premask(s))
                else:
                    hip.pool2d_bwd(g[s.dst], a[s.src], s.k, s.stride, s.ceil, s.mode, out=g[s.src],
                                   relu_mask_by_x=premask(s))
                cur = s.src
        if cur != 0:
            hip.fill_(g[0], 0.0)
        if self.ledger is not None:
            hip.loss_ledger_sum(self.ledger, self.slots_all, self.total, self.slots_f64)
            return
        if indep:
            for b in range(x.shape[0]):
                hip.sum_small(self.slots_all[b], self.total[b:b + 1])
            return
        hip.sum_small(self.slots_all, self.total)
        for s in self.steps:
            if id(s) in self.terms:
                t = self.terms[id(s)]
                self.slots_all[s.slot:s.slot + 1] = self.slots_all[t[0]:t[-1] + 1].sum(0, keepdim=True)

    def capture_content(self, x):
        self._prepare(x)
        a = self.act
        a[0] = x
        want = [s for s in self.steps if s.kind == "content" and "temporal" not in getattr(s.mod, "name", "")]
        last = max((self.steps.index(s) for s in want), default=-1)
        for s in self.steps[:last + 1]:
            if s.kind == "conv":
                if id(s) in self.fused_pool:
                    ps = self.fused_pool[id(s)]
                    models_mod.conv3x3_relu_pool(a[s.src], s.mod, a[ps.dst], self.pool_codes[id(ps)], workspace=self.ws)
                elif self.x6_fwd and self._x6_ok(s, s.mod.out_channels):
                    models_mod.conv3x3_mfma(a[s.src], s.mod, False, out=a[s.dst], relu=s.relu, workspace=self.ws)
                elif self.x6_fwd and models_mod.conv1x1_is_mfma(s.mod, False):
                    models_mod.conv1x1_mfma(a[s.src], s.mod, False, out=a[s.dst], relu=s.relu, workspace=self.ws)
                elif self.x6_fwd and models_mod.conv5x5_is_mfma(s.mod, False):
                    models_mod.conv5x5_mfma(a[s.src], s.mod, False, out=a[s.dst], relu=s.relu, workspace=self.ws)
                elif id(s) in self.strided_fwd_sites:
                    models_mod.conv_strided_fwd_as_3x3(a[s.src], s.mod, a[s.dst], s.relu, self.strided_fwd_sites[id(s)], workspace=self.ws)
                else:
                    wf, _ = s.mod.banks()
                    hip.conv2d_fwd(a[s.src], wf, s.mod.bias_device(), s.k, s.stride, s.pad, s.relu, out=a[s.dst],
                                   workspace=self.ws)
            elif s.kind == "relu":
                hip.relu_(a[s.src])
            elif s.kind == "pool":
                if id(s) not in self.pooled_by_conv:
                    hip.pool2d_fwd(a[s.src], s.k, s.stride, s.ceil, s.mode, out=a[s.dst])
        for s in want:
            t = getattr(s.mod, "target", None)
            if torch.is_tensor(t) and t.shape == a[s.src].shape and t.device == a[s.src].device and t.dtype == a[s.src].dtype:
                t.copy_(a[s.src])
            else:
                s.mod.target = a[s.src].detach().clone()

    def _graph_key(self):
        def sig(t):
            return None if t is None or not torch.is_tensor(t) else (t.data_ptr(), tuple(t.shape))
        key = []
        for s in self.steps:
            m = s.mod
            if s.kind in ("tv", "content", "style"):
                key.append((s.kind, id(m), getattr(m, "mode", None), float(m.strength), bool(getattr(m, "normalize", False)),
                            sig(getattr(m, "target", None)), sig(getattr(m, "video_target", None)), sig(getattr(m, "weights", None)),
                            float(getattr(m, "video_style_factor", 0.0)), bool(getattr(m, "use_covariance", False))))
            elif s.kind == "conv":
                key.append((id(m), m.weight.data_ptr(), m.weight._version))
        key.append(("hint", self.batch_hint, self.independent))
        return tuple(key)

    def feval(self, x, capture=False):
        self._prepare(x)
        if not capture:
            self._run(x)
            return self.slots, self.total, self.gbuf[0]
        key = self._graph_key()
        if self.graph is None or self.graph_key != key:
            self.graph, self.graph_key = None, key
            self.x_static.copy_(x)
            self._run(self.x_static)
            torch.cuda.synchronize()
            self.graph = torch.cuda.CUDAGraph()
            with torch.cuda.graph(self.graph):
                self._run(self.x_static)
        self.x_static.copy_(x)
        self.graph.replay()
        return self.slots, self.total, self.gbuf[0]

    def describe_routes(self, x, independent=None, batch_hint=None):
        assert models_mod.ROUTE_LOG is None, "describe_routes: a recording is already running"
        keep = (self.independent, self.batch_hint)
        if independent is not None:
            self.independent = bool(independent)
        if batch_hint is not None:
            self.batch_hint = int(batch_hint)
        models_mod.ROUTE_LOG = []
        try:
            self._prepare(x)
            self._run(x)
            torch.cuda.synchronize()
            log = models_mod.ROUTE_LOG
        finally:
            models_mod.ROUTE_LOG = None
            self.independent, self.batch_hint = keep
        return log

    def drop_graphs(self):
        self.iter_graphs = {}
        self.graph, self.graph_key = None, None

    def saved_bytes(self):
        tot = 0
        for d in (self.act, self.gbuf):
            for t in d.values():
                if t is not None and not t.is_meta:
                    tot += t.numel() * 4
        return tot
```

### maua-style_amd/hip.py

```python
import ctypes
import threading
import os
import sys

import torch

HERE = os.path.dirname(os.path.abspath(__file__))
LIB_PATH = os.path.join(HERE, "libmaua_hip.so")

c_f = ctypes.c_float
c_i = ctypes.c_int
c_i64 = ctypes.c_int64
c_p = ctypes.c_void_p
c_sz = ctypes.c_size_t
c_u64 = ctypes.c_uint64

SIGNATURES = {
    "maua_abi_version": (c_i, []),
    "maua_last_error": (ctypes.c_char_p, []),
    "maua_conv_pack_filters": (c_i, [c_p, c_p, c_p, c_i, c_i, c_i, c_i, c_p]),
    "maua_conv_workspace_bytes": (c_sz, [c_i, c_i, c_i, c_i, c_i, c_i, c_i, c_i, c_i]),
    "maua_conv2d_fwd": (c_i, [c_p, c_p, c_p, c_p, c_p, c_i, c_i, c_i, c_i, c_i, c_i, c_i, c_i, c_i, c_i, c_i, c_p, c_sz, c_p]),
    "maua_conv2d_bwd_data": (c_i, [c_p, c_p, c_p, c_p, c_p, c_p, c_i, c_i, c_i, c_i, c_i, c_i, c_i, c_i, c_i, c_i, c_p, c_sz,
                                   c_p]),
    "maua_conv_x6_bank_bytes": (c_sz, [c_i, c_i]),
    "maua_conv_pack_filters_x6": (c_i, [c_p, c_p, c_p, c_i, c_i, c_p]),
    "maua_conv_x6_workspace_bytes": (c_sz, [c_i, c_i, c_i, c_i, c_i, c_i]),
    "maua_conv_x3_bank_bytes": (c_sz, [c_i, c_i]),
    "maua_conv_pack_filters_x3": (c_i, [c_p, c_p, c_p, c_i, c_i, c_f, c_p]),
    "maua_conv_x3w_bank_bytes": (c_sz, [c_i, c_i]),
    "maua_conv_pack_filters_x3w": (c_i, [c_p, c_p, c_p, c_i, c_i, c_f, c_p]),
    "maua_conv_x3w_supported": (c_i, [c_i, c_i, c_i, c_i]),
    "maua_conv_x3w_workspace_bytes": (c_sz, [c_i, c_i, c_i, c_i, c_i, c_i]),
    "maua_conv3x3_x3w": (c_i, [c_p, c_p, c_f, c_p, c_p, c_p, c_i, c_i, c_i, c_i, c_i, c_i, c_i, c_i, c_p, c_sz, c_p]),
    "maua_conv_kxk_x3_bank_bytes": (c_sz, [c_i, c_i, c_i]),
    "maua_conv_pack_filters_kxk_x3": (c_i, [c_p, c_p, c_p, c_i, c_i, c_i, c_f, c_p]),
    "maua_conv_kxk_x3_workspace_bytes": (c_sz, [c_i, c_i, c_i, c_i, c_i, c_i, c_i]),
    "maua_conv_kxk_x3": (c_i, [c_p, c_p, c_f, c_p, c_p, c_p, c_i, c_i, c_i, c_i, c_i, c_i, c_i, c_i, c_i, c_p, c_sz, c_p]),
    "maua_conv1x1_x3_workspace_bytes": (c_sz, [c_i, c_i, c_i64, c_i]),
    "maua_conv1x1_x3": (c_i, [c_p, c_p, c_p, c_p, c_p, c_p, c_i, c_i, c_i64, c_i, c_i, c_i, c_p, c_sz, c_p]),
    "maua_conv_x3_workspace_bytes": (c_sz, [c_i, c_i, c_i, c_i, c_i, c_i]),
    "maua_conv3x3_x3": (c_i, [c_p, c_p, c_f, c_p, c_p, c_p, c_i, c_i, c_i, c_i, c_i, c_i, c_i, c_i, c_p, c_sz, c_p]),
    "maua_conv3x3_x6": (c_i, [c_p, c_p, c_p, c_p, c_p, c_i, c_i, c_i, c_i, c_i, c_i, c_i, c_i, c_p, c_sz, c_p]),
    "maua_conv_image_bank_bytes": (c_sz, [c_i, c_i]),
    "maua_conv_pack_filters_image": (c_i, [c_p, c_p, c_p, c_i, c_i, c_p]),
    "maua_conv3x3_image": (c_i, [c_p, c_p, c_p, c_i, c_i, c_i, c_i, c_i, c_i, c_i, c_p]),
    "maua_conv_image_gram_slabs": (c_i, [c_i, c_i, c_i]),
    "maua_conv_image_supported": (c_i, [c_i, c_i, c_i, c_i, c_i, c_i]),
    "maua_conv3x3_image_gram": (c_i, [c_p, c_p, c_p, c_p, c_i, c_i, c_i, c_i, c_p]),
    "maua_relu_fwd": (c_i, [c_p, c_i64, c_p]),
    "maua_relu_bwd": (c_i, [c_p, c_p, c_p, c_i64, c_p]),
    "maua_pool_out_size": (c_i, [c_i, c_i, c_i, c_i]),
    "maua_pool2d_fwd": (c_i, [c_p, c_p, c_i, c_i, c_i, c_i, c_i, c_i, c_i, c_i, c_p]),
    "maua_pool2d_bwd": (c_i, [c_p, c_p, c_p, c_i, c_i, c_i, c_i, c_i, c_i, c_i, c_i, c_i, c_p]),
    "maua_pool2x2_codes_supported": (c_i, [c_i, c_i, c_i, c_i]),
    "maua_pool2x2_fwd_codes": (c_i, [c_p, c_p, c_p, c_i, c_i, c_i, c_i, c_p]),
    "maua_pool2x2_bwd_codes": (c_i, [c_p, c_p, c_p, c_i, c_i, c_i, c_i, c_i, c_p]),
    "maua_gram_workspace_bytes": (c_sz, [c_i, c_i64]),
    "maua_gram_block": (c_i, [c_i, c_i64]),
    "maua_gram_fwd": (c_i, [c_p, c_p, c_p, c_i, c_i64, c_f, c_i, c_p, c_sz, c_p]),
    "maua_reduce_workspace_bytes": (c_sz, [c_i64]),
    "maua_mse_fwd_bwd": (c_i, [c_p, c_p, c_p, c_i64, c_f, c_f, c_i, c_i, c_p, c_p, c_sz, c_p]),
    "maua_mse_weighted_fwd_bwd": (c_i, [c_p, c_p, c_p, c_p, c_i64, c_i64, c_i, c_f, c_f, c_i, c_p, c_p, c_sz, c_p]),
    "maua_gram_bwd": (c_i, [c_p, c_p, c_p, c_p, c_p, c_i, c_i64, c_i, c_p, c_sz, c_p]),
    "maua_tv_fwd_bwd": (c_i, [c_p, c_p, c_i, c_i, c_i, c_i, c_f, c_i, c_p, c_p, c_sz, c_p]),
    "maua_fill": (c_i, [c_p, c_i64, c_f, c_p]),
    "maua_depth_to_space": (c_i, [c_p, c_p, c_i, c_i, c_i, c_i, c_i, c_i, c_i, c_i, c_p]),
    "maua_conv_few_mfma_bank_bytes": (c_sz, []),
    "maua_conv_pack_filters_few_mfma": (c_i, [c_p, c_p, c_i, c_i, c_p]),
    "maua_conv_few_mfma_supported": (c_i, [c_i, c_i, c_i, c_i, c_i, c_i]),
    "maua_conv3x3_few_mfma": (c_i, [c_p, c_p, c_p, c_i, c_i, c_i, c_i, c_i, c_i, c_p]),
    "maua_space_to_depth": (c_i, [c_p, c_p, c_i, c_i, c_i, c_i, c_i, c_i, c_i, c_p]),
    "maua_axpy": (c_i, [c_p, c_p, c_f, c_i64, c_p]),
    "maua_sum_small": (c_i, [c_p, c_i, c_p, c_p]),
    "maua_adam_step": (c_i, [c_p, c_p, c_p, c_p, c_i64, c_i, c_f, c_f, c_f, c_f, c_p]),
    "maua_channel_stats_workspace_bytes": (c_sz, [c_i, c_i]),
    "maua_channel_stats": (c_i, [c_p, c_p, c_f, c_i, c_i, c_i, c_i, c_p, c_p, c_sz, c_p]),
    "maua_color_match_solve": (c_i, [c_p, c_i, c_i64, c_p, c_i64, c_f, c_p, c_p]),
    "maua_color_match_apply": (c_i, [c_p, c_p, c_f, c_p, c_p, c_i, c_f, c_i, c_i, c_i, c_i, c_i, c_p, c_p]),
    "maua_resize_bilinear": (c_i, [c_p, c_p, c_i, c_i, c_i, c_i, c_i, c_f, c_f, c_p]),
    "maua_deprocess_u8": (c_i, [c_p, c_p, c_i, c_i, c_f, c_f, c_f, c_p]),
    "maua_set_tuning": (c_i, [ctypes.c_char_p, ctypes.c_double]),
    "maua_get_tuning": (ctypes.c_double, [ctypes.c_char_p, ctypes.c_double]),
    "maua_set_split_batch_hint": (None, [c_i]),
    "maua_conv_arm_workspace": (c_i, [c_p, c_p, c_sz, c_i, c_p]),
    "maua_get_split_batch_hint": (c_i, []),
    "maua_conv_x3w_split": (c_i, [c_i, c_i, c_i, c_i, c_i, c_i]),
    "maua_conv_x3q_bank_bytes": (c_sz, [c_i, c_i]),
    "maua_conv_pack_filters_x3q": (c_i, [c_p, c_p, c_p, c_i, c_i, c_f, c_p]),
    "maua_conv_x3q_supported": (c_i, [c_i, c_i, c_i, c_i]),
    "maua_conv_x3q_workspace_bytes": (c_sz, [c_i, c_i, c_i, c_i, c_i, c_i]),
    "maua_conv_x3q_split": (c_i, [c_i, c_i, c_i, c_i, c_i, c_i]),
    "maua_conv_x3q_preferred": (c_i, [c_i, c_i, c_i, c_i, c_i, c_i]),
    "maua_conv3x3_x3q": (c_i, [c_p, c_p, c_f, c_p, c_p, c_p, c_i, c_i, c_i, c_i, c_i, c_i, c_i, c_i, c_p, c_sz, c_p]),
    "maua_conv3x3_x3q_relu_pool": (c_i, [c_p, c_p, c_f, c_p, c_p, c_p, c_i, c_i, c_i, c_i, c_i, c_i, c_p, c_sz, c_p]),
    "maua_conv3x3_x3q_unpool": (c_i, [c_p, c_p, c_i, c_p, c_f, c_p, c_p, c_i, c_i, c_i, c_i, c_i, c_i, c_p, c_sz, c_p]),
    "maua_conv_x3p_supported": (c_i, [c_i, c_i, c_i, c_i, c_i]),
    "maua_conv_x3p_split": (c_i, [c_i, c_i, c_i, c_i, c_i, c_i]),
    "maua_conv_x3p_workspace_bytes": (c_sz, [c_i, c_i, c_i, c_i, c_i, c_i]),
    "maua_conv_x3p_preferred": (c_i, [c_i, c_i, c_i, c_i, c_i, c_i]),
    "maua_conv_x3p_set_max_groups": (c_i, [c_i]),
    "maua_conv3x3_x3p": (c_i, [c_p, c_p, c_i, c_p, c_f, c_p, c_p, c_p, c_p, c_p, c_p, c_i, c_i, c_i, c_i, c_i, c_i, c_i, c_p, c_sz, c_p]),
    "maua_conv3x3_x3w_relu_pool": (c_i, [c_p, c_p, c_f, c_p, c_p, c_p, c_i, c_i, c_i, c_i, c_i, c_i, c_p, c_sz, c_p]),
    "maua_conv_x3w_dmat_bank_bytes": (c_sz, [c_i]),
    "maua_conv_pack_dmat_x3w": (c_i, [c_p, c_i, c_p, c_p, c_p]),
    "maua_conv_pack_dmat_x3w_batch": (c_i, [c_i, c_p, c_p, c_p, c_p, c_p]),
    "maua_conv3x3_x3w_gram": (c_i, [c_p, c_p, c_f, c_p, c_p, c_p, c_p, c_i, c_i, c_i, c_i, c_i, c_i, c_i, c_p, c_sz, c_p]),
    "maua_conv3x3_x3w_unpool": (c_i, [c_p, c_p, c_i, c_p, c_f, c_p, c_p, c_p, c_p, c_i, c_i, c_i, c_i, c_i, c_i, c_p, c_sz, c_p]),
    "maua_loss_ledger_bytes": (c_sz, [c_i, c_i]),
    "maua_mse_fwd_bwd_ledger": (c_i, [c_p, c_p, c_p, c_i64, c_f, c_f, c_i, c_i, c_p, c_i, c_p]),
    "maua_tv_fwd_bwd_ledger": (c_i, [c_p, c_p, c_i, c_i, c_i, c_i, c_f, c_i, c_p, c_i, c_p]),
    "maua_gram_mse_ledger_supported": (c_i, [c_i]),
    "maua_gram_fwd_mse_ledger": (c_i, [c_p, c_p, c_p, c_i, c_i64, c_f, c_i, c_p, c_p, c_f, c_f, c_p, c_i, c_p, c_sz, c_p]),
    "maua_gram_partial": (c_i, [c_p, c_p, c_i, c_i64, c_i, c_p, c_sz, c_p]),
    "maua_gram_finish_mse_batch": (c_i, [c_i, c_p, c_p, c_p, c_p, c_p, c_p, c_p, c_p, c_p, c_p, c_p, c_p, c_p]),
    "maua_gram_partial_batch": (c_i, [c_i, c_p, c_p, c_p, c_p, c_p, c_p, c_p, c_p]),
    "maua_gram_row_means": (c_i, [c_p, c_p, c_i, c_i64, c_p, c_sz, c_p]),
    "maua_loss_ledger_sum": (c_i, [c_p, c_i, c_i, c_p, c_p, c_p]),
    "maua_loss_ledger_sum_f64": (c_i, [c_p, c_i, c_i, c_p, c_p, c_p, c_p]),
    "maua_lbfgs_state_bytes": (c_sz, [c_i64, c_i]),
    "maua_lbfgs_init": (c_i, [c_p, c_sz, c_i64, c_i, c_p]),
    "maua_lbfgs_iterate": (c_i, [c_p, c_p, c_p, c_p, c_i64, c_i, c_f, c_f, c_f, c_p]),
    "maua_lbfgs_status": (c_i, [c_p, c_i64, c_i, c_p, c_p]),
    "maua_flow_levels": (c_i, [c_i, c_i, c_i]),
    "maua_flow_grey_u8": (c_i, [c_p, c_p, c_i, c_i, c_p]),
    "maua_flow_pyr_down": (c_i, [c_p, c_p, c_i, c_i, c_p]),
    "maua_flow_warp_prep": (c_i, [c_p, c_p, c_p, c_p, c_i, c_i, c_p]),
    "maua_flow_tvl1_step": (c_i, [c_p, c_p, c_p, c_i, c_i, c_p]),
    "maua_flow_tvl1_blocked": (c_i, [c_p, c_p, c_p, c_i, c_i, c_i, c_p]),
    "maua_flow_median5": (c_i, [c_p, c_p, c_i, c_i, c_i, c_p]),
    "maua_flow_upsample": (c_i, [c_p, c_i, c_i, c_p, c_i, c_i, c_i, c_f, c_p]),
    "maua_flow_consistency_workspace_bytes": (c_sz, [c_i, c_i]),
    "maua_flow_consistency": (c_i, [c_p, c_p, c_p, c_i, c_i, c_p, c_sz, c_p]),
    "maua_flow_tvl1_workspace_bytes": (c_sz, [c_i, c_i, c_i]),
    "maua_flow_tvl1": (c_i, [c_p, c_p, c_p, c_i, c_i, c_i, c_i, c_i, c_i, c_p, c_sz, c_p]),
    "maua_nca_supported": (c_i, [c_i, c_i, c_i, c_i, c_i]),
    "maua_nca_param_count": (c_i64, [c_i, c_i]),
    "maua_nca_step": (c_i, [c_p, c_p, c_p, c_i, c_i, c_i, c_i, c_i, c_f, c_p, c_p, c_u64, c_i64, c_p]),
    "maua_nca_bwd_workspace_bytes": (c_sz, [c_i, c_i, c_i, c_i, c_i]),
    "maua_nca_step_bwd": (c_i, [c_p, c_p, c_p, c_p, c_i, c_i, c_i, c_i, c_i, c_f, c_p, c_p, c_u64, c_i64, c_i, c_p, c_sz, c_p]),
    "maua_nca_grad_finish": (c_i, [c_p, c_i, c_i, c_i, c_i, c_i, c_p, c_sz, c_i, c_p]),
}


class HipError(RuntimeError):
    pass


_lib = None


def lib():
    global _lib, LIB_PATH
    if _lib is None:
        LIB_PATH = os.environ.get("MAUA_HIP_LIB", LIB_PATH)
        if not os.path.exists(LIB_PATH):
            raise HipError(
                f"{LIB_PATH} not found: build it with `python maua-style_amd/build_native.py` "
                "(this package has no CPU or PyTorch fallback)")
        try:
            L = ctypes.CDLL(LIB_PATH)
        except OSError as e:
            raise HipError(f"cannot load {LIB_PATH}: {e}") from e
        for name, (res, args) in SIGNATURES.items():
            fn = getattr(L, name)
            fn.restype = res
            fn.argtypes = args
        _lib = L
        here = os.path.dirname(os.path.abspath(__file__))
        if here not in sys.path:
            sys.path.insert(0, here)
        import plan
        plan.forward_to_library(L)
        plan.warn_ignored()
    return _lib


def apply_plan():
    here = os.path.dirname(os.path.abspath(__file__))
    if here not in sys.path:
        sys.path.insert(0, here)
    import plan
    plan.forward_to_library(lib())


def _check(rc, what):
    if rc != 0:
        msg = lib().maua_last_error().decode(errors="replace")
        raise HipError(f"{what} failed (rc={rc}): {msg}")


def _ptr(t):
    if t is None:
        return None
    if not t.is_cuda:
        raise HipError("libmaua_hip needs ROCm device tensors (got a CPU tensor): there is no CPU path")
    if t.dtype != torch.float32 and t.dtype != torch.uint8 and t.dtype != torch.float64:
        raise HipError(f"unsupported dtype {t.dtype}")
    if not t.is_contiguous():
        raise HipError("tensor must be contiguous")
    return t.data_ptr()


def _stream():
    try:
        return torch._C._cuda_getCurrentRawStream(torch._C._cuda_getDevice())
    except AttributeError:
        return torch.cuda.current_stream().cuda_stream


def _f32(t, name):
    if t is not None and t.dtype != torch.float32:
        raise HipError(f"{name}: expected float32, got {t.dtype}")
    return t


def conv_pack_filters(w):
    cout, cin, kh, kw = w.shape
    wf = torch.empty(kh * kw, cin, cout, device=w.device, dtype=torch.float32)
    wb = torch.empty(kh * kw, cout, cin, device=w.device, dtype=torch.float32)
    _check(lib().maua_conv_pack_filters(_ptr(_f32(w, "w")), _ptr(wf), _ptr(wb), cout, cin, kh, kw, _stream()),
           "maua_conv_pack_filters")
    return wf, wb

# ... 488 lines not shown
    _check(lib().maua_gram_fwd_mse_ledger(_ptr(_f32(f, "f")), _ptr(out), _ptr(mean_out) if center else None, c, hw, float(scale),
                                          int(center), _ptr(_f32(target, "target")), _ptr(dmat), float(loss_scale),
                                          float(grad_scale), ledger.data_ptr(), int(slot), workspace.data_ptr(),
                                          workspace.numel() * workspace.element_size(), _stream()), "maua_gram_fwd_mse_ledger")
    return out


def gram_row_means(f, mean_out, workspace):
    c = f.shape[1] if f.dim() == 4 else f.shape[0]
    _check(lib().maua_gram_row_means(_ptr(_f32(f, "f")), _ptr(mean_out), c, f.numel() // c, workspace.data_ptr(),
                                     workspace.numel() * workspace.element_size(), _stream()), "maua_gram_row_means")


def gram_partial(f, center, mean_out, workspace):
    c = f.shape[1] if f.dim() == 4 else f.shape[0]
    hw = f.numel() // c
    _check(lib().maua_gram_partial(_ptr(_f32(f, "f")), _ptr(mean_out) if center else None, c, hw, int(center), workspace.data_ptr(),
                                   workspace.numel() * workspace.element_size(), _stream()), "maua_gram_partial")


class GramFinishBatch:

    def __init__(self, layers):
        n = len(layers)
        self.n = n
        self.keep = layers
        arr = lambda ct, vals: (ct * n)(*vals)
        self.args = (
            arr(ctypes.c_void_p, [l["workspace"].data_ptr() for l in layers]), arr(ctypes.c_void_p, [_ptr(l["gram"]) for l in layers]),
            arr(ctypes.c_void_p, [_ptr(_f32(l["target"], "target")) for l in layers]), arr(ctypes.c_void_p, [_ptr(l["dmat"]) for l in layers]),
            arr(ctypes.c_int, [int(l["c"]) for l in layers]), arr(ctypes.c_int64, [int(l["hw"]) for l in layers]),
            arr(ctypes.c_float, [float(l["scale"]) for l in layers]), arr(ctypes.c_float, [float(l["loss_scale"]) for l in layers]),
            arr(ctypes.c_float, [float(l["grad_scale"]) for l in layers]), arr(ctypes.c_void_p, [l["ledger"].data_ptr() for l in layers]),
            arr(ctypes.c_int, [int(l["slot"]) for l in layers]), arr(ctypes.c_int, [int(l.get("slabs") or 0) for l in layers]))

        self.partial_args = (
            arr(ctypes.c_void_p, [_ptr(_f32(l["f"], "f")) if l.get("f") is not None else None for l in layers]), self.args[4], self.args[5],
            self.args[0], arr(ctypes.c_size_t, [l["workspace"].numel() * l["workspace"].element_size() for l in layers]),
            arr(ctypes.c_void_p, [_ptr(l["mean"]) if l.get("mean") is not None else None for l in layers]))

    def run_partial(self):
        a = self.partial_args
        _check(lib().maua_gram_partial_batch(self.n, a[0], a[5], a[1], a[2], a[3], a[4], self.args[11], _stream()), "maua_gram_partial_batch")

    def run(self):
        a = self.args
        _check(lib().maua_gram_finish_mse_batch(self.n, a[0], a[1], a[2], a[3], a[4], a[5], a[6], a[7], a[8], a[9], a[10], a[11], _stream()),
               "maua_gram_finish_mse_batch")


def mse_fwd_bwd_ledger(x, target, grad, loss_scale, grad_scale, accumulate, ledger, slot, mask_grad_by_x=False):
    _check(lib().maua_mse_fwd_bwd_ledger(_ptr(_f32(x, "x")), _ptr(_f32(target, "target")), _ptr(grad), x.numel(), float(loss_scale),
                                         float(grad_scale), int(accumulate), int(mask_grad_by_x), ledger.data_ptr(), int(slot),
                                         _stream()), "maua_mse_fwd_bwd_ledger")


def tv_fwd_bwd_ledger(x, grad, strength, accumulate, ledger, slot):
    n, c, h, w = x.shape
    _check(lib().maua_tv_fwd_bwd_ledger(_ptr(_f32(x, "x")), _ptr(grad), n, c, h, w, float(strength), int(accumulate),
                                        ledger.data_ptr(), int(slot), _stream()), "maua_tv_fwd_bwd_ledger")


def loss_ledger_sum(ledger, losses, totals, losses_f64=None):
    frames, slots = ledger.shape[0], ledger.shape[1]
    if losses_f64 is not None:
        assert losses_f64.dtype == torch.float64 and losses_f64.numel() == frames * slots and losses_f64.is_contiguous()
        _check(lib().maua_loss_ledger_sum_f64(ledger.data_ptr(), frames, slots, _ptr(losses), _ptr(totals), losses_f64.data_ptr(),
                                              _stream()), "maua_loss_ledger_sum_f64")
        return
    _check(lib().maua_loss_ledger_sum(ledger.data_ptr(), frames, slots, _ptr(losses), _ptr(totals), _stream()),
           "maua_loss_ledger_sum")


def gram_bwd(d_sym, f, row_mean, gf, accumulate, workspace=None, relu_mask=None):
    c = d_sym.shape[0]
    hw = f.numel() // c
    workspace = _ws(workspace, 4 * c + 256, f.device)
    _check(lib().maua_gram_bwd(_ptr(_f32(d_sym, "d")), _ptr(f), _ptr(row_mean), _ptr(relu_mask), _ptr(gf), c, hw, int(accumulate),
                               workspace.data_ptr(), workspace.numel() * workspace.element_size(), _stream()),
           "maua_gram_bwd")
    return gf


def mse_fwd_bwd(x, target, grad, loss_scale, grad_scale, accumulate, loss_out, workspace=None, mask_grad_by_x=False):
    n = x.numel()
    workspace = _ws(workspace, reduce_workspace_bytes(n), x.device)
    _check(lib().maua_mse_fwd_bwd(_ptr(_f32(x, "x")), _ptr(_f32(target, "target")), _ptr(grad), n, float(loss_scale),
                                  float(grad_scale), int(accumulate), int(mask_grad_by_x), _ptr(loss_out),
                                  workspace.data_ptr(),
                                  workspace.numel() * workspace.element_size(), _stream()), "maua_mse_fwd_bwd")
    return loss_out


def mse_weighted_fwd_bwd(x, weights, target, grad, loss_scale, grad_scale, accumulate, loss_out, workspace=None):
    n, c, h, w = x.shape
    wplanes = weights.numel() // (h * w)
    workspace = _ws(workspace, reduce_workspace_bytes(x.numel()), x.device)
    _check(lib().maua_mse_weighted_fwd_bwd(_ptr(_f32(x, "x")), _ptr(_f32(weights, "weights")), _ptr(_f32(target, "target")),
                                           _ptr(grad), n * c, h * w, wplanes, float(loss_scale), float(grad_scale),
                                           int(accumulate), _ptr(loss_out), workspace.data_ptr(),
                                           workspace.numel() * workspace.element_size(), _stream()),
           "maua_mse_weighted_fwd_bwd")
    return grad


def tv_fwd_bwd(x, grad, strength, accumulate, loss_out, workspace=None):
    n, c, h, w = x.shape
    workspace = _ws(workspace, reduce_workspace_bytes(x.numel()), x.device)
    _check(lib().maua_tv_fwd_bwd(_ptr(_f32(x, "x")), _ptr(grad), n, c, h, w, float(strength), int(accumulate),
                                 _ptr(loss_out), workspace.data_ptr(), workspace.numel() * workspace.element_size(),
                                 _stream()), "maua_tv_fwd_bwd")
    return loss_out


def fill_(x, value):
    _check(lib().maua_fill(_ptr(x), x.numel(), float(value), _stream()), "maua_fill")
    return x


def axpy_(y, x, alpha):
    _check(lib().maua_axpy(_ptr(y), _ptr(x), float(alpha), x.numel(), _stream()), "maua_axpy")
    return y


def sum_small(slots, out):
    _check(lib().maua_sum_small(_ptr(slots), slots.numel(), _ptr(out), _stream()), "maua_sum_small")
    return out


def adam_step(x, grad, exp_avg, exp_avg_sq, step, lr, beta1=0.9, beta2=0.999, eps=1e-8):
    _check(lib().maua_adam_step(_ptr(x), _ptr(grad), _ptr(exp_avg), _ptr(exp_avg_sq), x.numel(), int(step), float(lr),
                                beta1, beta2, eps, _stream()), "maua_adam_step")


def conv_pack_filters_few_mfma(w):
    cout, cin = w.shape[:2]
    bank = torch.empty(lib().maua_conv_few_mfma_bank_bytes(), dtype=torch.uint8, device=w.device)
    _check(lib().maua_conv_pack_filters_few_mfma(_ptr(_f32(w, "w")), bank.data_ptr(), cout, cin, _stream()), "maua_conv_pack_filters_few_mfma")
    return bank


def conv_few_mfma_supported(n, cin, h, w, cout, pad):
    return bool(lib().maua_conv_few_mfma_supported(int(n), int(cin), int(h), int(w), int(cout), int(pad)))


def conv3x3_few_mfma(gy, bank, cin, out=None, tile=0):
    n, cout, h, w = gy.shape
    if out is None:
        out = torch.empty(n, cin, h, w, device=gy.device, dtype=torch.float32)
    _check(lib().maua_conv3x3_few_mfma(_ptr(_f32(gy, "gy")), bank.data_ptr(), _ptr(out), n, cin, h, w, cout, int(tile), _stream()), "maua_conv3x3_few_mfma")
    return out


def space_to_depth(x, r, out):
    n, c, h, w = x.shape
    assert out.shape[0] == n and out.shape[1] == r * r * c
    _check(lib().maua_space_to_depth(_ptr(_f32(x, "x")), _ptr(out), n, c, r, h, w, out.shape[2], out.shape[3], _stream()), "maua_space_to_depth")
    return out


def depth_to_space(x, r, out, accumulate=False):
    n, cc, qh, qw = x.shape
    c_out = out.shape[1]
    assert cc == r * r * c_out and out.shape[0] == n
    _check(lib().maua_depth_to_space(_ptr(_f32(x, "x")), _ptr(out), n, c_out, r, qh, qw, out.shape[2], out.shape[3], int(accumulate), _stream()),
           "maua_depth_to_space")
    return out


ARRIVAL_COUNTER_BYTES = 4096 * 4
_ARMED = threading.local()


def conv_arm_workspace(workspace, counters=None, zero=True):
    if workspace is None:
        _check(lib().maua_conv_arm_workspace(None, None, 0, 0, _stream()), "maua_conv_arm_workspace")
        _ARMED.pair = None
        return None
    if counters is None:
        counters = torch.empty(ARRIVAL_COUNTER_BYTES, dtype=torch.uint8, device=workspace.device)
        zero = True
    _check(lib().maua_conv_arm_workspace(workspace.data_ptr(), counters.data_ptr(), counters.numel() * counters.element_size(), int(bool(zero)),
                                         _stream()), "maua_conv_arm_workspace")
    _ARMED.pair = (workspace, counters)
    return counters


def set_split_batch_hint(frames):
    prev = lib().maua_get_split_batch_hint()
    lib().maua_set_split_batch_hint(int(frames))
    return prev


def channel_stats(x, noise=None, noise_amp=1e-3, out=None, workspace=None):
    b, c, h, w = x.shape
    if c != 3:
        raise HipError("channel_stats: 3-channel images")
    if out is None:
        out = torch.empty(b, 9, dtype=torch.float64, device=x.device)
    workspace = _ws(workspace, lib().maua_channel_stats_workspace_bytes(h, w), x.device)
    if noise is not None and noise.numel() != x.numel():
        raise HipError("channel_stats: noise must have the batch's element count")
    for j in range(b):
        _check(lib().maua_channel_stats(_ptr(_f32(x, "x")), _ptr(noise), float(noise_amp), b, j, h, w, _ptr(out[j]),
                                        workspace.data_ptr(), workspace.numel() * workspace.element_size(), _stream()),
               "maua_channel_stats")
    return out


def color_match_solve(stats_t, pixels_t, stats_s, pixels_s, eps, coef_out):
    _check(lib().maua_color_match_solve(_ptr(stats_t), stats_t.shape[0], int(pixels_t), _ptr(stats_s), int(pixels_s), float(eps),
                                        _ptr(coef_out), _stream()), "maua_color_match_solve")
    return coef_out


def color_match_apply(x, noise, noise_amp, coef, all_coef, weight, accumulate, out):
    b, c, h, w = x.shape
    for j in range(b):
        _check(lib().maua_color_match_apply(_ptr(_f32(x, "x")), _ptr(noise), float(noise_amp), _ptr(coef), _ptr(all_coef),
                                            all_coef.numel() // 16, float(weight), int(accumulate), b, j, h, w, _ptr(out), _stream()),
               "maua_color_match_apply")
    return out


def resize_bilinear(x, size=None, scale_factor=None):
    import math
    import numpy as np
    n, c, h, w = x.shape
    if (size is None) == (scale_factor is None):
        raise HipError("resize_bilinear: give exactly one of size / scale_factor")
    if scale_factor is not None:
        oh, ow = int(math.floor(float(h) * scale_factor)), int(math.floor(float(w) * scale_factor))
        sh = sw = float(np.float32(1.0 / scale_factor))
    else:
        oh, ow = (int(size), int(size)) if isinstance(size, int) else (int(size[0]), int(size[1]))
        sh, sw = float(np.float32(h) / np.float32(oh)), float(np.float32(w) / np.float32(ow))
    if oh <= 0 or ow <= 0:
        raise HipError(f"resize_bilinear: output {oh}x{ow}")
    out = torch.empty(n, c, oh, ow, device=x.device, dtype=torch.float32)
    _check(lib().maua_resize_bilinear(_ptr(_f32(x, "x")), _ptr(out), n * c, h, w, oh, ow, sh, sw, _stream()), "maua_resize_bilinear")
    return out


def deprocess_u8(x, mean_bgr):
    x3 = x.reshape(3, x.shape[-2], x.shape[-1])
    _, h, w = x3.shape
    out = torch.empty(h, w, 3, dtype=torch.uint8, device=x.device)
    _check(lib().maua_deprocess_u8(_ptr(_f32(x3, "x")), out.data_ptr(), h, w, float(mean_bgr[0]), float(mean_bgr[1]),
                                   float(mean_bgr[2]), _stream()), "maua_deprocess_u8")
    return out


class LbfgsState:

    def __init__(self, count, history, device):
        self.count, self.history = int(count), int(history)
        if not 0 < self.history <= 254:
            raise HipError(f"--lbfgs_num_correction {history}: the device-side recursion holds at most 254 pairs")
        nbytes = lib().maua_lbfgs_state_bytes(self.count, self.history)
        self.buf = torch.empty(nbytes, dtype=torch.uint8, device=device)
        self._status = torch.zeros(5, dtype=torch.float32, device=device)
        _check(lib().maua_lbfgs_init(self.buf.data_ptr(), nbytes, self.count, self.history, _stream()), "maua_lbfgs_init")

    def reset(self):
        _check(lib().maua_lbfgs_init(self.buf.data_ptr(), self.buf.numel(), self.count, self.history, _stream()), "maua_lbfgs_init")

    def iterate(self, x, grad, lr=1.0, tolerance_change=-1.0, tolerance_grad=-1.0, loss=None):
        _check(lib().maua_lbfgs_iterate(self.buf.data_ptr(), _ptr(x), _ptr(grad), _ptr(loss), self.count, self.history, float(lr),
                                        float(tolerance_change), float(tolerance_grad), _stream()), "maua_lbfgs_iterate")

    def status(self):
        _check(lib().maua_lbfgs_status(self.buf.data_ptr(), self.count, self.history, _ptr(self._status), _stream()),
               "maua_lbfgs_status")
        n_iter, hlen, stopped, gtd, t = self._status.tolist()
        return dict(n_iter=int(n_iter), history_len=int(hlen), stopped=bool(stopped), gtd=gtd, t=t)


FLOW_MAX_LEVELS = 8


def _flow_dims_ok(h, w):
    return 0 < h <= 1 << 16 and 0 < w <= 1 << 16 and h * w <= 1 << 28


def flow_levels(h, w, max_levels=5):
    if not _flow_dims_ok(h, w) or max_levels < 1:
        return 0
    n = 1
    while n < max_levels and (h + 1) // 2 >= 16 and (w + 1) // 2 >= 16:
        h, w, n = (h + 1) // 2, (w + 1) // 2, n + 1
    return n


def flow_tvl1_workspace_bytes(h, w, levels):
    if not _flow_dims_ok(h, w) or not 1 <= levels <= FLOW_MAX_LEVELS or levels > flow_levels(h, w, levels):
        return 0
    a = lambda b: (b + 255) & ~255
    total, lh, lw = 0, h, w
    for _ in range(levels):
        total += 2 * a(lh * lw * 4)
        lh, lw = (lh + 1) // 2, (lw + 1) // 2
    return total + 2 * a(6 * h * w * 4) + a(3 * h * w * 4) + a(2 * h * w * 4)


def _u8(t, name, shape=None):
    if not t.is_cuda or t.dtype != torch.uint8 or not t.is_contiguous():
# ... 156 lines not shown
```

### maua-style_amd/models.py

```python
import copy
from os import path

import torch
import torch.nn as nn

import hip
import plan
from loss import ContentLoss, GramMatrix, ScaleGradients, StyleLoss, TVLoss


ROUTE_LOG = None


def _route(kernel, x, produced, pad, backward, tile, ksplit=1, **fused):
    if ROUTE_LOG is not None:
        rec = {"kernel": kernel, "pass": "bwd" if backward else "fwd", "consumed": int(x.shape[1]), "produced": int(produced),
               "plane": [int(x.shape[2]), int(x.shape[3])], "n": int(x.shape[0]), "pad": int(pad), "tile": tile, "ksplit": int(ksplit)}
        rec.update({k: v for k, v in fused.items() if v})
        ROUTE_LOG.append(rec)



def _x6_mode():
    mode = plan.get("conv_x6")
# ... 22 lines not shown
    return int(v) if v.isdigit() else 64


def conv3x3_is_x3p(consumed, h, w, pad, produced, n=1, accumulate=False):
    mc = _x3p_min_channels()
    return _x3_enabled() and _x3w_enabled() and mc > 0 and mc <= consumed <= plan.get_int("conv_x3p_max") and not accumulate and h * w >= _x3w_min_pixels() and \
        hip.conv_x3p_supported(consumed, h, w, produced, pad) and hip.conv_x3p_preferred(n, consumed, h, w, produced, pad)


def _x3p_gram_enabled(n, c_in, c_out, h, w):
    mb = hip.lib().maua_get_split_batch_hint() * (c_in + 2 * c_out) * h * w * 4 / 1e6
    return mb >= plan.get_float("x3p_gram_min_mb")


X3Q_UNPOOL_MIN_CHANNELS = 512


def conv3x3_is_x3q(consumed, h, w, pad, at_least=0, produced=None, n=1):
    mc = max(_x3q_min_channels(), at_least) if _x3q_min_channels() > 0 else 0
    return _x3_enabled() and _x3w_enabled() and mc > 0 and consumed >= mc and h * w >= _x3w_min_pixels() and \
        hip.conv_x3q_supported(consumed, h, w, pad) and (produced is None or hip.conv_x3q_preferred(n, consumed, h, w, produced, pad))


def _x3w_min_pixels():
    return plan.get_int("x3w_min_pixels")


def conv3x3_mfma(x, mod, backward, out=None, out_relu_mask=None, relu=False, accumulate=False, workspace=None, pool_group=False):
    pad = mod.padding[0]
    if backward:
        cout, p, bias = mod.in_channels, 2 - pad, None
    else:
        cout, p, bias = mod.out_channels, pad, mod.bias_device()
    consumed = mod.out_channels if backward else mod.in_channels
    n, h, w = x.shape[0], x.shape[2], x.shape[3]
    if conv3x3_is_x3p(consumed, x.shape[2], x.shape[3], p, cout, x.shape[0], accumulate):
        bf, bb, wsc = mod.banks3q()
        _route("conv_x3p", x, cout, p, backward, "64co x 16x32px, persistent", hip.conv_x3p_split(n, consumed, h, w, cout, p) if workspace is not None else 1,
               mask=out_relu_mask is not None, relu=relu)
        return hip.conv3x3_x3p(x, bb if backward else bf, wsc, bias, cout, p, relu, out=out, out_relu_mask=out_relu_mask, workspace=workspace)
    if conv3x3_is_x3q(consumed, x.shape[2], x.shape[3], p, X3Q_UNPOOL_MIN_CHANNELS if pool_group else 0, cout, x.shape[0]):
        bf, bb, wsc = mod.banks3q()
        _route("conv_x3q", x, cout, p, backward, "64co x 16x32px", hip.conv_x3q_split(n, consumed, h, w, cout, p) if workspace is not None else 1,
               mask=out_relu_mask is not None, relu=relu, accumulate=accumulate)
        return hip.conv3x3_x3q(x, bb if backward else bf, wsc, bias, cout, p, relu, out=out, out_relu_mask=out_relu_mask,
                               accumulate=accumulate, workspace=workspace)
    if _x3_enabled() and _x3w_enabled() and x.shape[2] * x.shape[3] >= _x3w_min_pixels() and \
            hip.conv_x3w_supported(consumed, x.shape[2], x.shape[3], p):
        bf, bb, wsc = mod.banks3w()
        _route("conv_x3w", x, cout, p, backward, "64co x 8x32px", hip.conv_x3w_split(n, consumed, h, w, cout, p) if workspace is not None else 1,
               mask=out_relu_mask is not None, relu=relu, accumulate=accumulate)
        return hip.conv3x3_x3w(x, bb if backward else bf, wsc, bias, cout, p, relu, out=out, out_relu_mask=out_relu_mask,
                               accumulate=accumulate, workspace=workspace)
    if _x3_enabled() and consumed > 4:
        bf, bb, wsc = mod.banks3()
        _route("conv_x3", x, cout, p, backward, "64co x 4x32px", mask=out_relu_mask is not None, relu=relu, accumulate=accumulate)
        return hip.conv3x3_x3(x, bb if backward else bf, wsc, bias, cout, p, relu, out=out, out_relu_mask=out_relu_mask,
                              accumulate=accumulate, workspace=workspace)
    if not backward and consumed <= 3 and out_relu_mask is None and not accumulate and _image_kernel_enabled() and \
            hip.conv_image_supported(n, consumed, h, w, cout, p):
        _route("conv_image", x, cout, p, backward, "27 (channel, tap) pairs as K, bf16x6", relu=relu)
        return hip.conv3x3_image(x, mod.bank_image(), cout, p, relu, out=out)
    bf, bb = mod.banks6()
    _route("conv_x6" if cout > 4 or consumed < 16 else "conv3x3_few_out", x, cout, p, backward, "bf16x6", mask=out_relu_mask is not None, relu=relu, accumulate=accumulate)
    return hip.conv3x3_x6(x, bb if backward else bf, bias, cout, p, relu, out=out, out_relu_mask=out_relu_mask,
                          accumulate=accumulate, workspace=workspace)


def conv3x3_fwd_is_x3w(mod, h, w):
    return _x3_enabled() and _x3w_enabled() and h * w >= _x3w_min_pixels() and mod.kernel_size[0] == 3 and mod.stride[0] == 1 and \
        hip.conv_x3w_supported(mod.in_channels, h, w, mod.padding[0])


def conv3x3_fwd_family(mod, n, h, w):
    cin, cout, pad = mod.in_channels, mod.out_channels, mod.padding[0]
    if conv3x3_is_x3p(cin, h, w, pad, cout, n):
        return "conv_x3p", hip.conv_x3p_split(n, cin, h, w, cout, pad)
    if conv3x3_is_x3q(cin, h, w, pad, 0, cout, n):
        return "conv_x3q", hip.conv_x3q_split(n, cin, h, w, cout, pad)
    return "conv_x3w", hip.conv_x3w_split(n, cin, h, w, cout, pad)


def conv3x3_relu_pool(x, mod, pooled, codes, workspace=None):
    if conv3x3_is_x3p(mod.in_channels, x.shape[2], x.shape[3], mod.padding[0], mod.out_channels, x.shape[0]):
        bf, _, wsc = mod.banks3q()
        _route("conv_x3p", x, mod.out_channels, mod.padding[0], False, "64co x 16x32px, persistent",
               hip.conv_x3p_split(x.shape[0], mod.in_channels, x.shape[2], x.shape[3], mod.out_channels, mod.padding[0]) if workspace is not None else 1, relu=True, pool=True)
        return hip.conv3x3_x3p(x, bf, wsc, mod.bias_device(), mod.out_channels, mod.padding[0], True, out=pooled, pool_codes=codes,
                               workspace=workspace)
    if conv3x3_is_x3q(mod.in_channels, x.shape[2], x.shape[3], mod.padding[0], 0, mod.out_channels, x.shape[0]):
        bf, _, wsc = mod.banks3q()
        _route("conv_x3q", x, mod.out_channels, mod.padding[0], False, "64co x 16x32px",
               hip.conv_x3q_split(x.shape[0], mod.in_channels, x.shape[2], x.shape[3], mod.out_channels, mod.padding[0]) if workspace is not None else 1, relu=True, pool=True)
        return hip.conv3x3_x3q_relu_pool(x, bf, wsc, mod.bias_device(), mod.out_channels, mod.padding[0], pooled, codes, workspace=workspace)
    bf, _, wsc = mod.banks3w()
    _route("conv_x3w", x, mod.out_channels, mod.padding[0], False, "64co x 8x32px",
           hip.conv_x3w_split(x.shape[0], mod.in_channels, x.shape[2], x.shape[3], mod.out_channels, mod.padding[0]) if workspace is not None else 1, relu=True, pool=True)
    return hip.conv3x3_x3w_relu_pool(x, bf, wsc, mod.bias_device(), mod.out_channels, mod.padding[0], pooled, codes, workspace=workspace)


def conv3x3_bwd_is_x3w(mod, h, w):
    pad = mod.padding[0]
    return _x3_enabled() and _x3w_enabled() and h * w >= _x3w_min_pixels() and mod.kernel_size[0] == 3 and mod.stride[0] == 1 and \
        hip.conv_x3w_supported(mod.out_channels, h, w, 2 - pad)


def conv3x3_bwd_with_gram(gy, mod, feature_map, dmat_bank, dmat_inv_scale, out, workspace=None):
    if conv3x3_is_x3p(mod.out_channels, gy.shape[2], gy.shape[3], 2 - mod.padding[0], mod.in_channels, gy.shape[0]) and \
            _x3p_gram_enabled(gy.shape[0], mod.out_channels, mod.in_channels, gy.shape[2], gy.shape[3]):
        _, bb, wsc = mod.banks3q()
        _route("conv_x3p", gy, mod.in_channels, 2 - mod.padding[0], True, "64co x 16x32px, persistent", mask=True, gram=True)
        return hip.conv3x3_x3p(gy, bb, wsc, None, mod.in_channels, 2 - mod.padding[0], False, out=out, out_relu_mask=feature_map,
                               dmat_bank=dmat_bank, dmat_inv_scale=dmat_inv_scale, workspace=workspace)
    _, bb, wsc = mod.banks3w()
    _route("conv_x3w", gy, mod.in_channels, 2 - mod.padding[0], True, "64co x 8x32px",
           hip.conv_x3w_split(gy.shape[0], mod.out_channels, gy.shape[2], gy.shape[3], mod.in_channels, 2 - mod.padding[0]) if workspace is not None else 1, mask=True, gram=True)
    return hip.conv3x3_x3w_gram(gy, bb, wsc, feature_map, dmat_bank, dmat_inv_scale, mod.in_channels, 2 - mod.padding[0], out=out,
                                workspace=workspace)


def conv3x3_bwd_from_pooled(gy_pooled, codes, honour_relu_bit, mod, out, out_relu_mask=None, dmat_bank=None, dmat_inv_scale=None,
                            workspace=None):
    if conv3x3_is_x3p(mod.out_channels, out.shape[2], out.shape[3], 2 - mod.padding[0], mod.in_channels, gy_pooled.shape[0]) and \
            (dmat_bank is None or _x3p_gram_enabled(out.shape[0], mod.out_channels // 4, mod.in_channels, out.shape[2], out.shape[3])):
        _, bb, wsc = mod.banks3q()
        _route("conv_x3p", out, mod.in_channels, 2 - mod.padding[0], True, "64co x 16x32px, persistent", mask=out_relu_mask is not None, unpool=True, gram=dmat_bank is not None)
        return hip.conv3x3_x3p(gy_pooled, bb, wsc, None, mod.in_channels, 2 - mod.padding[0], False, out=out, out_relu_mask=out_relu_mask,
                               in_codes=codes, honour_relu_bit=honour_relu_bit, dmat_bank=dmat_bank, dmat_inv_scale=dmat_inv_scale,
                               workspace=workspace)
    if dmat_bank is None and conv3x3_is_x3q(mod.out_channels, out.shape[2], out.shape[3], 2 - mod.padding[0], X3Q_UNPOOL_MIN_CHANNELS,
                                            mod.in_channels, gy_pooled.shape[0]):
        _, bb, wsc = mod.banks3q()
        _route("conv_x3q", out, mod.in_channels, 2 - mod.padding[0], True, "64co x 16x32px", mask=out_relu_mask is not None, unpool=True)
        return hip.conv3x3_x3q_unpool(gy_pooled, codes, honour_relu_bit, bb, wsc, mod.in_channels, 2 - mod.padding[0], out=out,
                                      out_relu_mask=out_relu_mask, workspace=workspace)
    _, bb, wsc = mod.banks3w()
    _route("conv_x3w", out, mod.in_channels, 2 - mod.padding[0], True, "64co x 8x32px", mask=out_relu_mask is not None, unpool=True, gram=dmat_bank is not None)
    return hip.conv3x3_x3w_unpool(gy_pooled, codes, honour_relu_bit, bb, wsc, mod.in_channels, 2 - mod.padding[0], out=out,
                                  out_relu_mask=out_relu_mask, dmat_bank=dmat_bank, dmat_inv_scale=dmat_inv_scale, workspace=workspace)


def conv_strided_bwd_is_3x3(mod, h_out, w_out):
    k, stride, pad = mod.kernel_size[0], mod.stride[0], mod.padding[0]
    return plan.on("strided_bwd_3x3") and _x6_mode()[1] and _x3_enabled() and _x3w_enabled() and stride > 1 and pad == 0 and k <= 3 * stride and \
        stride * stride * mod.in_channels <= 64 and mod.out_channels % 16 == 0 and (h_out + 2) * (w_out + 2) >= _x3w_min_pixels() and \
        hip.conv_x3w_supported(mod.out_channels, h_out, w_out, 2)


def conv_few_is_mfma(mod, n, h, w):
    k, stride, pad = mod.kernel_size[0], mod.stride[0], mod.padding[0]
    return plan.on("few_mfma") and _x6_mode()[1] and k == 3 and stride == 1 and pad == 1 and hip.conv_few_mfma_supported(n, mod.in_channels, h, w, mod.out_channels, pad)


def conv_few_mfma(gy, mod, out):
    _route("conv_few_mfma", gy, mod.in_channels, 1, True, "4 / 8 x 62 px, bf16x6")
    return hip.conv3x3_few_mfma(gy, mod.bank_few_mfma(), mod.in_channels, out=out)


def conv_strided_fwd_is_3x3(mod, h, w):
    k, stride, pad = mod.kernel_size[0], mod.stride[0], mod.padding[0]
    if not (plan.on("strided_fwd_3x3") and _x6_mode()[0] and _x3_enabled() and _x3w_enabled() and stride > 1 and pad == 0 and k <= 3 * stride and
            (stride * stride * mod.in_channels) % 16 == 0 and mod.out_channels > 32 and h >= k and w >= k):
        return False
    qh, qw = (h - k) // stride + 3, (w - k) // stride + 3
    return qh * qw >= _x3w_min_pixels() and bool(hip.conv_x3w_supported(stride * stride * mod.in_channels, qh, qw, 0))


def conv_strided_fwd_as_3x3(x, mod, out, relu, sites, workspace=None):
    s_ = mod.stride[0]
    hip.space_to_depth(x, s_, sites)
    bank, wsc = mod.bank_strided_fwd()
    _route("conv_x3w", sites, mod.out_channels, 0, False, "64co x 8x32px", 1, strided_as_3x3=True, relu=relu)
    return hip.conv3x3_x3w(sites, bank, wsc, mod.bias_device(), mod.out_channels, 0, relu, out=out, workspace=workspace)


def conv_strided_bwd_as_3x3(gy, mod, out, workspace=None, sites=None):
    s_, c_img = mod.stride[0], mod.in_channels
    bank, wsc = mod.bank_strided_bwd()
    sites = hip.conv3x3_x3w(gy, bank, wsc, None, s_ * s_ * c_img, 2, False, out=sites, workspace=workspace)
    _route("conv_x3w", gy, s_ * s_ * c_img, 2, True, "64co x 8x32px", 1, strided_as_3x3=True)
    return hip.depth_to_space(sites, s_, out)


def conv1x1_is_mfma(mod, backward):
    k, stride, pad = mod.kernel_size[0], mod.stride[0], mod.padding[0]
    produced = mod.in_channels if backward else mod.out_channels
    return _x6_mode()[1 if backward else 0] and _x3_enabled() and k == 1 and stride == 1 and pad == 0 and produced > 32


def conv1x1_mfma(x, mod, backward, out=None, out_relu_mask=None, relu=False, workspace=None):
    w2d, w2d_t = mod.mats()
    _route("conv1x1_x3", x, mod.in_channels if backward else mod.out_channels, 0, backward, "64co x 128px", mask=out_relu_mask is not None, relu=relu)
    if backward:
        return hip.conv1x1_x3(x, w2d_t, None, False, out=out, out_relu_mask=out_relu_mask, workspace=workspace)
    return hip.conv1x1_x3(x, w2d, mod.bias_device(), relu, out=out, out_relu_mask=out_relu_mask, workspace=workspace)


def conv5x5_is_mfma(mod, backward):
    k, stride, pad = mod.kernel_size[0], mod.stride[0], mod.padding[0]
    produced = mod.in_channels if backward else mod.out_channels
    return _x6_mode()[1 if backward else 0] and _x3_enabled() and k == 5 and stride == 1 and pad <= 4 and produced > 32


def conv5x5_mfma(x, mod, backward, out=None, out_relu_mask=None, relu=False, workspace=None):
    bf, bb, wsc = mod.banks_kxk()
    k, pad = mod.kernel_size[0], mod.padding[0]
    _route("conv_kxk_x3", x, mod.in_channels if backward else mod.out_channels, k - 1 - pad if backward else pad, backward, "k x k, fp16x3", mask=out_relu_mask is not None, relu=relu)
    if backward:
        return hip.conv_kxk_x3(x, bb, wsc, None, mod.in_channels, k, k - 1 - pad, False, out=out, out_relu_mask=out_relu_mask,
                               workspace=workspace)
    return hip.conv_kxk_x3(x, bf, wsc, mod.bias_device(), mod.out_channels, k, pad, relu, out=out, out_relu_mask=out_relu_mask,
                           workspace=workspace)


class _ConvFn(torch.autograd.Function):
    @staticmethod
    def forward(ctx, x, mod):
        ctx.mod, ctx.in_shape = mod, x.shape
        k, stride, pad = mod.kernel_size[0], mod.stride[0], mod.padding[0]
        if _x6_mode()[0] and k == 3 and stride == 1 and pad <= 2 and mod.out_channels >= plan.get_int("split_min_produced"):
            return conv3x3_mfma(x.contiguous(), mod, False)
        if conv1x1_is_mfma(mod, False):
            return conv1x1_mfma(x.contiguous(), mod, False)
        if conv5x5_is_mfma(mod, False):
            return conv5x5_mfma(x.contiguous(), mod, False)
        return hip.conv2d_fwd(x.contiguous(), mod.banks()[0], mod.bias_device(), k, stride, pad, False)

    @staticmethod
    def backward(ctx, gy):
        mod = ctx.mod
        k, stride, pad = mod.kernel_size[0], mod.stride[0], mod.padding[0]
        if _x6_mode()[1] and k == 3 and stride == 1 and pad <= 2 and mod.in_channels >= plan.get_int("split_min_produced"):
            return conv3x3_mfma(gy.contiguous(), mod, True), None
        if conv1x1_is_mfma(mod, True):
            return conv1x1_mfma(gy.contiguous(), mod, True), None
        if conv5x5_is_mfma(mod, True):
            return conv5x5_mfma(gy.contiguous(), mod, True), None
        gx = hip.conv2d_bwd_data(gy.contiguous(), None, mod.banks()[1], mod.weight.detach(), ctx.in_shape, k, stride, pad)
        return gx, None


class Conv2d(nn.Conv2d):

    def reset_parameters(self):
        pass

    def banks(self):
        key = (self.weight.data_ptr(), self.weight._version, self.weight.device)
        if getattr(self, "_bank_key", None) != key:
            self._banks = hip.conv_pack_filters(self.weight.detach().contiguous())
            self._bank_key = key
        return self._banks

    def bank_image(self):
        b = self.bias_device()
        key = (self.weight.data_ptr(), self.weight._version, self.weight.device, None if b is None else (b.data_ptr(), b._version))
        if getattr(self, "_bank_img_key", None) != key:
            self._bank_img = hip.conv_pack_filters_image(self.weight.detach().contiguous(), b)
            self._bank_img_key = key
        return self._bank_img

    def banks6(self):
        key = (self.weight.data_ptr(), self.weight._version, self.weight.device)
        if getattr(self, "_bank6_key", None) != key:
            self._banks6 = hip.conv_pack_filters_x6(self.weight.detach().contiguous())
            self._bank6_key = key
        return self._banks6

    def banks3(self):
        key = (self.weight.data_ptr(), self.weight._version, self.weight.device)
        if getattr(self, "_bank3_key", None) != key:
            self._banks3 = hip.conv_pack_filters_x3(self.weight.detach().contiguous())
            self._bank3_key = key
        return self._banks3

    def banks3w(self):
        key = (self.weight.data_ptr(), self.weight._version, self.weight.device)
        if getattr(self, "_bank3w_key", None) != key:
            self._banks3w = hip.conv_pack_filters_x3w(self.weight.detach().contiguous())
            self._bank3w_key = key
        return self._banks3w

    def banks3q(self):
        key = (self.weight.data_ptr(), self.weight._version, self.weight.device)
        if getattr(self, "_bank3q_key", None) != key:
            self._banks3q = hip.conv_pack_filters_x3q(self.weight.detach().contiguous())
            self._bank3q_key = key
        return self._banks3q

    def bank_few_mfma(self):
        key = (self.weight.data_ptr(), self.weight._version, self.weight.device)
        if getattr(self, "_bankfm_key", None) != key:
            self._bankfm = hip.conv_pack_filters_few_mfma(self.weight.detach().contiguous())
            self._bankfm_key = key
        return self._bankfm

    def bank_strided_fwd(self):
        key = (self.weight.data_ptr(), self.weight._version, self.weight.device)
        if getattr(self, "_banksf_key", None) != key:
            w = self.weight.detach()
            co, ci, k, _ = w.shape
            s_ = self.stride[0]
            wp = torch.zeros(co, ci, 3 * s_, 3 * s_, device=w.device, dtype=w.dtype)
            wp[:, :, :k, :k] = w
            f = wp.view(co, ci, 3, s_, 3, s_).permute(0, 3, 5, 1, 2, 4).reshape(co, s_ * s_ * ci, 3, 3).contiguous()
            bank, _, wsc = hip.conv_pack_filters_x3w(f)
# ... 331 lines not shown
```

### maua-style_amd/plan.py

```python
import os
import sys

FIELDS = {
    "conv_x6": ("1", "host", "3x3 stride-1 layers on the reduced-width matrix cores with fp32-accurate operand splits: 1 both passes, fwd / bwd one pass, 0 fp32 MFMA"),
    "conv_x3": ("1", "host", "1: fp16x3 arithmetic (22 significand bits, conv_x3*.hip); 0: bf16x6 everywhere (the strictly 24-bit route bench.py reports beside the headline)"),
    "conv_x3w": ("1", "host", "layers whose consumed channel count is a multiple of 16 run conv_x3w.hip instead of conv_x3.hip"),
    "conv_x3q": ("256", "host", "smallest consumed channel count from which a 3x3 layer runs conv_x3q.hip (0: never)"),
    "conv_x3p": ("64", "host", "smallest consumed channel count from which a 3x3 layer may run the persistent conv_x3p.hip (0: never); conv_x3p_preferred decides per launch"),
    "conv_x3p_max": ("100000", "host", "largest consumed channel count for conv_x3p.hip"),
    "x3p_gram_min_mb": ("700", "host", "the Gram backward rides in conv_x3p's launch from this many MB of maps per launch (below: conv_x3w's fused form)"),
    "conv_image": ("1", "host", "the 3-channel image layer's forward pass on conv_img.hip"),
    "split_min_produced": ("16", "host", "a 3x3 stride-1 pass runs the split-precision kernels (64-channel tiles) when it PRODUCES at least this many channels, else the fp32-MFMA / direct kernels (VGG-19 / NIN: only the 64 -> 3 image gradient is below; the pruned VGG-16 has widths of 22 and 24)"),
    "x3w_min_pixels": ("4096", "host", "planes smaller than this run conv_x3.hip's 4-row tiles"),
    "few_mfma": ("1", "host", "backward-data of the image layer (64 -> 3 channels) on the matrix cores (conv_few_mfma.hip) instead of conv3x3_few_out's vector-ALU kernel"),
    "strided_fwd_3x3": ("1", "host", "forward pass of a strided, unpadded layer (NIN's stem) as space to depth + a stride-1 3x3 convolution over sites (conv_x3w)"),
    "strided_bwd_3x3": ("1", "host", "backward-data of a strided, unpadded layer (NIN's 11x11 / 4 stem) as a stride-1 3x3 convolution over the output sites + depth to space"),
    "pool_codes": ("1", "host", "2x2 / 2 max pools keep one decision byte per window for the backward pass"),
    "loss_ledger": ("1", "host", "loss partial sums go to a ledger summed once per evaluation"),
    "gram_batch": ("1", "host", "one finishing launch for the Gram / loss chains of all style layers"),
    "gram_partial_batch": ("1", "host", "one partial-product launch for the Gram-form layers"),
    "fuse_pool": ("1", "host", "conv + ReLU + pool in one launch where the pool is the activation's only consumer"),
    "fuse_pool_split": ("1", "host", "... also where the small grid splits the channel loop (the adding pass pools)"),
    "fuse_unpool": ("1", "host", "backward-data staged straight from the pooled map's gradient and the decision bytes"),
    "fuse_gram_max_c": ("256", "host", "style layers of at most this many channels have their Gram backward ride in the next convolution's backward launch (0: never)"),
    "image_gram": ("1", "host", "the image layer's launch leaves the Gram slabs of relu1_1"),
    "finish_in_launch": ("0", "host", "1: the engine arms its split-K workspace - small splits are added up by the last workgroup to arrive at a tile, no finishing launch (bit-identical; measured neutral at 512 x 512: the last arriver's serial chain costs what the launch cost, profiles/probes_r06.md section 1)"),
    "dmat_pack_batch": ("1", "host", "one launch packs the D matrices of all fused style layers"),
    "style_stream": ("auto", "host", "Gram / loss chains of a single image on a side stream: 0, 1, or auto (from 1536 x 1536 pixels)"),
    "side_streams": ("4", "host", "side streams for the per-frame kernels of independent frames (0: none)"),
    "hip_graph": ("1", "host", "replay iterations from captured hipGraphs"),
    "graph_bundles": ("1", "host", "L-BFGS iterations captured as whole bundles (evaluation + update)"),
    "frame_batch": ("0", "host", "vid_img: frames per batch (0: planned from memory; 1: the reference's frame-by-frame loop)"),
    "frame_cache_mb": ("4096", "host", "vid_img: host cache for decoded frames"),
    "debug_poison": ("0", "host", "tests: every engine buffer starts as NaN"),
    "conv_few_out": ("1", "lib", "3x3 passes that produce <= 4 channels run conv3x3_few_out (0: the general MFMA kernel)"),
    "few_out_ks4_below": ("1024", "lib", "conv3x3_few_out: launches of fewer workgroups than this split the channel loop four ways"),
    "x3w_ks": ("0", "lib", "conv_x3w: force this K split (0: cost model)"),
    "x3w_stagger": ("7", "lib", "conv_x3w: start delay of odd-slot workgroups, units of 512 cycles"),
    "finish_in_launch_max_ks": ("4", "lib", "split channel loops of at most this many slabs are finished inside the producing launch when the workspace is armed (conv_x3q, conv_x3w)"),
    "x3q_ks": ("0", "lib", "conv_x3q: force this K split (0: cost model)"),
    "x3q_min_fill": ("0.85", "lib", "conv_x3q_preferred: smallest grid fill x plane cover"),
    "x3q_min_chunks": ("4", "lib", "conv_x3q_preferred: smallest number of 32-channel chunks per workgroup"),
    "x3p_ks": ("0", "lib", "conv_x3p: force this K split (0: cost model)"),
    "cot_inner": ("0", "lib", "conv_x3w / conv_x3q workgroup order: 1 = the channel tiles of a pixel tile start side by side on one XCD (shared patch in its L2), 0 = blockIdx.y is the channel tile"),
    "x3p_order": ("1", "lib", "conv_x3p's work list: 0 channel tile outermost (an XCD's band = part of one channel tile's plane), 1 pixel tile outermost (the channel tiles of a pixel tile side by side on an XCD's CUs: the plane leaves memory once)"),
    "x3p_groups": ("256", "lib", "conv_x3p: workgroups per launch (a multiple of 8)"),
    "x3p_min_fill": ("0.8", "lib", "conv_x3p_preferred: smallest list fill x plane cover"),
    "x3p_min_items": ("512", "lib", "conv_x3p_preferred: smallest number of work items (and a quarter of the smallest items x chunks)"),
    "x6_persist": ("0", "lib", "conv_x6: several tiles per workgroup (experiment)"),
    "gram_x3": ("1", "lib", "Gram partial products in fp16x3 (0: fp32 MFMA)"),
    "gram_bwd_x3": ("1", "lib", "Gram backward in fp16x3 (0: fp32 MFMA)"),
    "gram_t128": ("1", "lib", "128 x 128 two-role Gram blocks: 0 never, 1 whole 64-pixel stages, 2 ragged maps too"),
    "gram_t128_min_hw": ("1024", "lib", "128 x 128 Gram blocks from this many pixels"),
    "p1_order": ("1", "lib", "conv1x1_x3: (pixel tile, channel tile) items in XCD bands, channel tiles adjacent (0: dispatch order)"),
    "lbfgs_vec": ("1", "lib", "lbfgs: 16-byte loads in the history sweeps"),
    "lbfgs_tri": ("1", "lib", "lbfgs: the triangular form of the coefficient kernel"),
}

ENV_VARS = {
    "MAUA_HIP_LIB": None,
    "MAUA_PLAN": None,
    "MAUA_CONV_X3": "conv_x3",
    "MAUA_CONV_X6": "conv_x6",
    "MAUA_HIP_GRAPH": "hip_graph",
    "MAUA_DEBUG_POISON": "debug_poison",
    "MAUA_DIST_BACKEND": None,
    "MAUA_DIST_TIMEOUT_S": None,
    "MAUA_DIST_JOB_TIMEOUT_S": None,
    "MAUA_HOST_THREADS": None,
}
_FIELD_VAR = {field: var for var, field in ENV_VARS.items() if field is not None}
_TOOL_VARS = {"MAUA_FUZZ_ASSUME_NO_GPU"}

OVERRIDES = {}


_plan_cache = (None, {})


def _planned():
    global _plan_cache
    text = os.environ.get("MAUA_PLAN")
    if _plan_cache[0] != text or text is None:
        _plan_cache = (text, _parse_plan(text))
    return _plan_cache[1]


def _parse_plan(text):
    out = {}
    for part in (text or "").replace(";", ",").split(","):
        part = part.strip()
        if not part:
            continue
        if "=" not in part:
            raise ValueError(f"MAUA_PLAN: expected field=value, got {part!r}")
        k, v = part.split("=", 1)
        k = k.strip().lower()
        if k.startswith("maua_"):
            k = k[5:]
        if k not in FIELDS:
            raise ValueError(f"MAUA_PLAN: unknown field {k!r} (plan.FIELDS lists them)")
        out[k] = v.strip()
    return out


def get(name):
    default = FIELDS[name][0]
    if name in OVERRIDES:
        return str(OVERRIDES[name])
    planned = _planned()
    if name in planned:
        return planned[name]
    var = _FIELD_VAR.get(name)
    if var is not None and var in os.environ:
        return os.environ[var]
    return default


def get_int(name):
    return int(float(get(name)))


def get_float(name):
    return float(get(name))


def on(name):
    return get(name) != "0"


def in_effect():
    return {k: get(k) for k in FIELDS if get(k) != FIELDS[k][0]}


def ignored_variables(environ=None):
    environ = os.environ if environ is None else environ
    return sorted(k for k in environ if k.startswith("MAUA_") and k not in ENV_VARS and k not in _TOOL_VARS)


def env_overrides(environ=None):
    return {"in_effect": in_effect(), "ignored": ignored_variables(environ)}


_warned = False


def warn_ignored():
    global _warned
    ign = ignored_variables()
    if ign and not _warned:
        _warned = True
        hint = ",".join(f"{k[5:].lower()}={os.environ[k]}" for k in ign if k[5:].lower() in FIELDS)
        sys.stderr.write(f"maua: ignoring {', '.join(ign)} (not among the honoured variables {sorted(ENV_VARS)})"
                         + (f"; use MAUA_PLAN=\"{hint}\"" if hint else "") + "\n")
    return ign


def forward_to_library(lib):
    for k, (default, who, _) in FIELDS.items():
        if who == "lib":
            rc = lib.maua_set_tuning(k.encode(), float(get(k)))
            if rc != 0:
                raise RuntimeError(f"libmaua_hip does not know the tuning constant {k!r}")
```

Before: 200.5.

## Fuse TV loss into the image-layer backward few-MFMA epilogue

The total-variation loss gradient and its loss partials are now computed in the epilogue of the 64->3 image-layer backward-data kernel, so the separate TV launch is skipped and gx is not re-read and re-written. The kernel also becomes persistent-capable: each workgroup can walk several tiles of its XCD band and prefetch the next tile's loads, which is needed to bound ledger partials per launch. Non-temporal load and store options are added behind tuning knobs that are off by default. The fused path adds neighbour reads of x plus a double-precision block reduction into the ledger, and it caps the grid size when the ledger limits it.

```diff
diff --git a/include/maua_hip.h b/include/maua_hip.h
--- a/include/maua_hip.h
+++ b/include/maua_hip.h
@@ -179,6 +179,9 @@
 int maua_conv_pack_filters_few_mfma(const float* w_oihw, void* bank, int cout, int cin, maua_stream_t stream);
 int maua_conv_few_mfma_supported(int n, int cin, int h, int w, int cout, int pad);
 int maua_conv3x3_few_mfma(const float* gy, const void* bank, float* gx, int n, int cin, int h, int w, int cout, int tile, maua_stream_t stream);
+int maua_conv_few_mfma_tv_supported(int n, int cin, int h, int w, int cout, int pad);
+int maua_conv3x3_few_mfma_tv(const float* gy, const void* bank, float* gx, const float* x, int n, int cin, int h, int w, int cout, int tile,
+                             float strength, double* ledger, int slot, maua_stream_t stream);
 
 int maua_space_to_depth(const float* in, float* out, int n, int c_in, int r, int h, int w, int qh, int qw, maua_stream_t stream);
 int maua_depth_to_space(const float* in, float* out, int n, int c_out, int r, int qh, int qw, int h, int w, int accumulate, maua_stream_t stream);
diff --git a/maua-style_amd/csrc/conv_api.hip b/maua-style_amd/csrc/conv_api.hip
--- a/maua-style_amd/csrc/conv_api.hip
+++ b/maua-style_amd/csrc/conv_api.hip
@@ -16,7 +16,8 @@
 namespace maua {
 static const char* const g_tuning_names[] = {"conv_few_out", "few_out_ks4_below", "x3w_ks", "x3w_stagger", "x3q_ks", "x3q_min_fill", "x3q_min_chunks",
                                              "x3p_ks", "x3p_groups", "x3p_min_fill", "x3p_min_items", "x6_persist", "gram_x3", "gram_bwd_x3",
-                                             "gram_t128", "gram_t128_min_hw", "p1_order", "lbfgs_vec", "lbfgs_tri", "finish_in_launch_max_ks", "x3p_order", "cot_inner"};
+                                             "gram_t128", "gram_t128_min_hw", "p1_order", "lbfgs_vec", "lbfgs_tri", "finish_in_launch_max_ks", "x3p_order", "cot_inner",
+                                             "few_mfma_groups", "few_mfma_nt", "image_nt"};
 constexpr int kTunings = sizeof(g_tuning_names) / sizeof(g_tuning_names[0]);
 static double g_tuning_values[kTunings];
 static bool g_tuning_set[kTunings];
diff --git a/maua-style_amd/csrc/conv_few_mfma.hip b/maua-style_amd/csrc/conv_few_mfma.hip
--- a/maua-style_amd/csrc/conv_few_mfma.hip
+++ b/maua-style_amd/csrc/conv_few_mfma.hip
@@ -47,18 +47,26 @@
     float* gx;
     int H, W, co;
     int tiles_x, tiles, per_xcd;
+    const float* x;
+    float strength;
+    double* rec;
 };
 
-template <int ROWS>
+template <int ROWS, bool TV, bool NT>
 __global__ void __launch_bounds__(256, 2) conv_few_mfma_kernel(FewMfmaArgs p) {
     extern __shared__ float T[];
+    __shared__ double scratch[16];
     constexpr int TR = ROWS + 2, TPL = TR * FM_TC, NBLK = TR * 2;
+    constexpr int AUX = NT ? 2 : 0;
     const int tid = threadIdx.x, lane = tid & 63, wave = tid >> 6, nl = lane & 31, kg = lane >> 5;
-    const int tile = (int)(blockIdx.x & 7) * p.per_xcd + (int)(blockIdx.x >> 3);
-    if (tile >= p.tiles) return;
-    const int ty = tile / p.tiles_x;
-    const int x0 = (tile - ty * p.tiles_x) * FM_OC, y0 = ty * ROWS, img = blockIdx.z;
+    const int xcd = (int)(blockIdx.x & 7), wpx = (int)(gridDim.x >> 3), img = blockIdx.z;
+    const int band = min(p.per_xcd, p.tiles - xcd * p.per_xcd);
     const int64_t plane = (int64_t)p.H * p.W;
+    double tv_acc = 0.0;
+    if (TV && blockIdx.x == 0 && blockIdx.z == 0 && tid == 0) {
+        p.rec[0] = (double)(gridDim.x * gridDim.z);
+        p.rec[1] = (double)p.strength;
+    }
     fm_bf16x8 a[FM_STEPS][3];
 #pragma unroll
     for (int step = 0; step < FM_STEPS; ++step)
@@ -67,7 +75,7 @@
             a[step][part] = *reinterpret_cast<const fm_bf16x8*>(p.bank + (((step * 3 + part) * 64) + lane) * 16);
     const __amdgpu_buffer_rsrc_t rs = __builtin_amdgcn_make_buffer_rsrc(const_cast<float*>(p.gy) + (int64_t)img * FM_K * plane, 0,
                                                                         (unsigned)(FM_K * plane * 4), 0x00020000);
-    auto request = [&](float (&v)[FM_STEPS][8], int b) {
+    auto request = [&](float (&v)[FM_STEPS][8], int b, int x0, int y0) {
         const int tr = b >> 1, Y = y0 - 1 + tr, X = x0 - 1 + 32 * (b & 1) + nl;
         const bool ok = Y >= 0 && Y < p.H && X >= 0 && X < p.W;
         const unsigned voff = ok ? (unsigned)(((int64_t)kg * 8 * plane + (int64_t)Y * p.W + X) * 4) : 0x80000000u;
@@ -75,70 +83,150 @@
         for (int step = 0; step < FM_STEPS; ++step)
 #pragma unroll
             for (int i = 0; i < 8; ++i)
-                v[step][i] = __builtin_bit_cast(float, __builtin_amdgcn_raw_buffer_load_b32(rs, voff, (unsigned)((16 * step + i) * plane * 4), 0));
+                v[step][i] = __builtin_bit_cast(float, __builtin_amdgcn_raw_buffer_load_b32(rs, voff, (unsigned)((16 * step + i) * plane * 4), AUX));
+    };
+    auto origin = [&](int j, int& x0, int& y0) {
+        const int tile = xcd * p.per_xcd + j, ty = tile / p.tiles_x;
+        x0 = (tile - ty * p.tiles_x) * FM_OC;
+        y0 = ty * ROWS;
     };
     float v[FM_STEPS][8], vn[FM_STEPS][8];
-    if (wave < NBLK) request(v, wave);
-    for (int b = wave; b < NBLK; b += 4) {
-        if (b + 4 < NBLK) request(vn, b + 4);
-        fm_f32x16 acc;
-#pragma unroll
-        for (int r = 0; r < 16; ++r) acc[r] = 0.f;
-#pragma unroll
-        for (int step = 0; step < FM_STEPS; ++step) {
-            fm_u32x4 bp[3];
-#pragma unroll
-            for (int q = 0; q < 4; ++q) {
-                const float u0 = v[step][2 * q], u1 = v[step][2 * q + 1];
-                const unsigned h = fm_cvt_pk(u0, u1);
-                const float r0 = u0 - __builtin_bit_cast(float, h << 16), r1 = u1 - __builtin_bit_cast(float, h & 0xffff0000u);
-                const unsigned m = fm_cvt_pk(r0, r1);
-                const unsigned l = fm_cvt_pk(r0 - __builtin_bit_cast(float, m << 16), r1 - __builtin_bit_cast(float, m & 0xffff0000u));
-                bp[0][q] = h;
-                bp[1][q] = m;
-                bp[2][q] = l;
+    int x0 = 0, y0 = 0;
+    const int j0 = (int)(blockIdx.x >> 3);
+    if (j0 < band) {
+        origin(j0, x0, y0);
+        request(v, wave, x0, y0);
+    }
+    for (int j = j0; j < band; j += wpx) {
+        int nx0 = 0, ny0 = 0;
+        const bool more = j + wpx < band;
+        if (more) origin(j + wpx, nx0, ny0);
+        for (int b = wave; b < NBLK; b += 4) {
+            if (b + 4 < NBLK) request(vn, b + 4, x0, y0);
+            else if (more) request(vn, wave, nx0, ny0);
+            fm_f32x16 acc;
+#pragma unroll
+            for (int r = 0; r < 16; ++r) acc[r] = 0.f;
+#pragma unroll
+            for (int step = 0; step < FM_STEPS; ++step) {
+                fm_u32x4 bp[3];
+#pragma unroll
+                for (int q = 0; q < 4; ++q) {
+                    const float u0 = v[step][2 * q], u1 = v[step][2 * q + 1];
+                    const unsigned h = fm_cvt_pk(u0, u1);
+                    const float r0 = u0 - __builtin_bit_cast(float, h << 16), r1 = u1 - __builtin_bit_cast(float, h & 0xffff0000u);
+                    const unsigned m = fm_cvt_pk(r0, r1);
+                    const unsigned l = fm_cvt_pk(r0 - __builtin_bit_cast(float, m << 16), r1 - __builtin_bit_cast(float, m & 0xffff0000u));
+                    bp[0][q] = h;
+                    bp[1][q] = m;
+                    bp[2][q] = l;
+                }
+                const fm_bf16x8 b0v = __builtin_bit_cast(fm_bf16x8, bp[0]), b1v = __builtin_bit_cast(fm_bf16x8, bp[1]),
+                                b2v = __builtin_bit_cast(fm_bf16x8, bp[2]);
+                acc = __builtin_amdgcn_mfma_f32_32x32x16_bf16(a[step][2], b0v, acc, 0, 0, 0);
+                acc = __builtin_amdgcn_mfma_f32_32x32x16_bf16(a[step][1], b1v, acc, 0, 0, 0);
+                acc = __builtin_amdgcn_mfma_f32_32x32x16_bf16(a[step][0], b2v, acc, 0, 0, 0);
+                acc = __builtin_amdgcn_mfma_f32_32x32x16_bf16(a[step][1], b0v, acc, 0, 0, 0);
+                acc = __builtin_amdgcn_mfma_f32_32x32x16_bf16(a[step][0], b1v, acc, 0, 0, 0);
+                acc = __builtin_amdgcn_mfma_f32_32x32x16_bf16(a[step][0], b0v, acc, 0, 0, 0);
             }
-            const fm_bf16x8 b0v = __builtin_bit_cast(fm_bf16x8, bp[0]), b1v = __builtin_bit_cast(fm_bf16x8, bp[1]),
-                            b2v = __builtin_bit_cast(fm_bf16x8, bp[2]);
-            acc = __builtin_amdgcn_mfma_f32_32x32x16_bf16(a[step][2], b0v, acc, 0, 0, 0);
-            acc = __builtin_amdgcn_mfma_f32_32x32x16_bf16(a[step][1], b1v, acc, 0, 0, 0);
-            acc = __builtin_amdgcn_mfma_f32_32x32x16_bf16(a[step][0], b2v, acc, 0, 0, 0);
-            acc = __builtin_amdgcn_mfma_f32_32x32x16_bf16(a[step][1], b0v, acc, 0, 0, 0);
-            acc = __builtin_amdgcn_mfma_f32_32x32x16_bf16(a[step][0], b1v, acc, 0, 0, 0);
-            acc = __builtin_amdgcn_mfma_f32_32x32x16_bf16(a[step][0], b0v, acc, 0, 0, 0);
+            float* dst = T + (b >> 1) * FM_TC + 32 * (b & 1) + nl;
+#pragma unroll
+            for (int r = 0; r < 16; ++r) {
+                const int m = (r & 3) + 8 * (r >> 2) + 4 * kg;
+                if (m < 9 * p.co) dst[m * TPL] = acc[r];
+            }
+#pragma unroll
+            for (int step = 0; step < FM_STEPS; ++step)
+#pragma unroll
+                for (int i = 0; i < 8; ++i) v[step][i] = vn[step][i];
         }
-        float* dst = T + (b >> 1) * FM_TC + 32 * (b & 1) + nl;
-#pragma unroll
-        for (int r = 0; r < 16; ++r) {
-            const int m = (r & 3) + 8 * (r >> 2) + 4 * kg;
-            if (m < 9 * p.co) dst[m * TPL] = acc[r];
+        __syncthreads();
+        const int co = p.co;
+        for (int idx = tid; idx < ROWS * FM_OC; idx += 256) {
+            const int i = idx / FM_OC, jx = idx - i * FM_OC;
+            const int Y = y0 + i, X = x0 + jx;
+            if (Y >= p.H || X >= p.W) continue;
+            const float* t0 = T + (i + 2) * FM_TC + jx + 2;
+            for (int c = 0; c < co; ++c) {
+                float s = 0.f;
+#pragma unroll
+                for (int ky = 0; ky < 3; ++ky)
+#pragma unroll
+                    for (int kx = 0; kx < 3; ++kx) s += t0[((ky * 3 + kx) * co + c) * TPL - ky * FM_TC - kx];
+                const int64_t e = ((int64_t)img * co + c) * plane + (int64_t)Y * p.W + X;
+                if constexpr (TV) {
+                    const float* __restrict__ xp = p.x + e;
+                    const int W = p.W;
+                    auto sgn = [](float d) { return d > 0.f ? 1.f : (d < 0.f ? -1.f : 0.f); };
+                    const float cv = xp[0];
+                    const float dn = Y + 1 < p.H ? xp[W] : cv, up = Y > 0 ? xp[-W] : cv, rt = X + 1 < W ? xp[1] : cv, lf = X > 0 ? xp[-1] : cv;
+                    float g = 0.f;
+                    if (Y + 1 < p.H) {
+                        const float d = dn - cv;
+                        tv_acc += fabs((double)d);
+                        g -= sgn(d);
+                    }
+                    if (Y > 0) g += sgn(cv - up);
+                    if (X + 1 < W) {
+                        const float d = rt - cv;
+                        tv_acc += fabs((double)d);
+                        g -= sgn(d);
+                    }
+                    if (X > 0) g += sgn(cv - lf);
+                    s = fmaf(p.strength, g, s);
+                }
+                p.gx[e] = s;
+            }
         }
-#pragma unroll
-        for (int step = 0; step < FM_STEPS; ++step)
-#pragma unroll
-            for (int i = 0; i < 8; ++i) v[step][i] = vn[step][i];
-    }
-    __syncthreads();
-    const int co = p.co;
-    for (int idx = tid; idx < ROWS * FM_OC; idx += 256) {
-        const int i = idx / FM_OC, j = idx - i * FM_OC;
-        const int Y = y0 + i, X = x0 + j;
-        if (Y >= p.H || X >= p.W) continue;
-        const float* t0 = T + (i + 2) * FM_TC + j + 2;
-        for (int c = 0; c < co; ++c) {
-            float s = 0.f;
-#pragma unroll
-            for (int ky = 0; ky < 3; ++ky)
-#pragma unroll
-                for (int kx = 0; kx < 3; ++kx) s += t0[((ky * 3 + kx) * co + c) * TPL - ky * FM_TC - kx];
-            p.gx[((int64_t)img * co + c) * plane + (int64_t)Y * p.W + X] = s;
-        }
+        if (more) __syncthreads();
+        x0 = nx0;
+        y0 = ny0;
+    }
+    if constexpr (TV) {
+        tv_acc = block_sum(tv_acc, scratch);
+        if (tid == 0) p.rec[2 + (int64_t)blockIdx.z * gridDim.x + blockIdx.x] = tv_acc;
     }
 }
 
 }
 
 using namespace maua;
+
+template <int ROWS>
+static void few_mfma_launch(const FewMfmaArgs& p, bool tv, bool nt, dim3 grid, hipStream_t stream) {
+    const int lds = 27 * (ROWS + 2) * FM_TC * 4;
+    static unsigned long long attr[4] = {0, 0, 0, 0};
+#define FM_LAUNCH(TV, NT, SLOT)                                                                                            \
+    do {                                                                                                                   \
+        (void)opt_in_dynamic_lds(reinterpret_cast<const void*>(conv_few_mfma_kernel<ROWS, TV, NT>), lds, &attr[SLOT]);     \
+        hipLaunchKernelGGL((conv_few_mfma_kernel<ROWS, TV, NT>), grid, dim3(256), lds, stream, p);                         \
+    } while (0)
+    if (tv && nt) FM_LAUNCH(true, true, 0);
+    else if (tv) FM_LAUNCH(true, false, 1);
+    else if (nt) FM_LAUNCH(false, true, 2);
+    else FM_LAUNCH(false, false, 3);
+#undef FM_LAUNCH
+}
+
+static int few_mfma_run(FewMfmaArgs p, int n, int h, int w, int tile, bool tv, int max_groups, hipStream_t stream) {
+    if (tile == 0) tile = (int64_t)h * w < 1000000 ? 1 : 2;
+    const int rows = tile == 1 ? 4 : tile == 2 ? 8 : 14;
+    p.tiles_x = (w + FM_OC - 1) / FM_OC;
+    p.tiles = p.tiles_x * ((h + rows - 1) / rows);
+    p.per_xcd = (p.tiles + 7) / 8;
+    int wpx = p.per_xcd;
+    const int want = (int)tuning("few_mfma_groups", 0);
+    if (want >= 8 && want / 8 < wpx) wpx = want / 8;
+    if (max_groups > 0 && max_groups / 8 < wpx) wpx = max_groups / 8;
+    MAUA_REQUIRE(wpx >= 1, MAUA_E_UNSUPPORTED, "conv3x3_few_mfma_tv: %d images leave no room for a workgroup per XCD in the ledger record", n);
+    const dim3 grid((unsigned)(8 * wpx), 1, (unsigned)n);
+    const bool nt = tuning("few_mfma_nt", 0) != 0;
+    if (rows == 4) few_mfma_launch<4>(p, tv, nt, grid, stream);
+    else if (rows == 8) few_mfma_launch<8>(p, tv, nt, grid, stream);
+    else few_mfma_launch<14>(p, tv, nt, grid, stream);
+    return check_launch("conv_few_mfma_kernel");
+}
 
 extern "C" {
 
@@ -160,26 +248,21 @@
     MAUA_REQUIRE(gy && bank && gx, MAUA_E_INVAL, "conv3x3_few_mfma: null pointer");
     MAUA_REQUIRE(maua_conv_few_mfma_supported(n, cin, h, w, cout, 1), MAUA_E_UNSUPPORTED, "conv3x3_few_mfma: unsupported geometry");
     MAUA_REQUIRE(tile >= 0 && tile <= 3, MAUA_E_INVAL, "conv3x3_few_mfma: tile code 0 - 3");
-    if (tile == 0) tile = (int64_t)h * w < 1000000 ? 1 : 2;
-    FewMfmaArgs p{gy, (const unsigned char*)bank, gx, h, w, cin, 0, 0, 0};
-    static unsigned long long attr[4] = {0, 0, 0, 0};
-    const int rows = tile == 1 ? 4 : tile == 2 ? 8 : 14;
-    const int lds = 27 * (rows + 2) * FM_TC * 4;
-    p.tiles_x = (w + FM_OC - 1) / FM_OC;
-    p.tiles = p.tiles_x * ((h + rows - 1) / rows);
-    p.per_xcd = (p.tiles + 7) / 8;
-    const dim3 grid((unsigned)(8 * p.per_xcd), 1, (unsigned)n);
-    if (rows == 4) {
-        (void)opt_in_dynamic_lds(reinterpret_cast<const void*>(conv_few_mfma_kernel<4>), lds, &attr[1]);
-        hipLaunchKernelGGL(conv_few_mfma_kernel<4>, grid, dim3(256), lds, (hipStream_t)stream, p);
-    } else if (rows == 8) {
-        (void)opt_in_dynamic_lds(reinterpret_cast<const void*>(conv_few_mfma_kernel<8>), lds, &attr[2]);
-        hipLaunchKernelGGL(conv_few_mfma_kernel<8>, grid, dim3(256), lds, (hipStream_t)stream, p);
-    } else {
-        (void)opt_in_dynamic_lds(reinterpret_cast<const void*>(conv_few_mfma_kernel<14>), lds, &attr[3]);
-        hipLaunchKernelGGL(conv_few_mfma_kernel<14>, grid, dim3(256), lds, (hipStream_t)stream, p);
-    }
-    return check_launch("conv_few_mfma_kernel");
-}
-
-}
+    FewMfmaArgs p{gy, (const unsigned char*)bank, gx, h, w, cin, 0, 0, 0, nullptr, 0.f, nullptr};
+    return few_mfma_run(p, n, h, w, tile, false, 0, (hipStream_t)stream);
+}
+
+int maua_conv_few_mfma_tv_supported(int n, int cin, int h, int w, int cout, int pad) {
+    return maua_conv_few_mfma_supported(n, cin, h, w, cout, pad) && n <= LEDGER_MAX / 8;
+}
+
+int maua_conv3x3_few_mfma_tv(const float* gy, const void* bank, float* gx, const float* x, int n, int cin, int h, int w, int cout, int tile,
+                             float strength, double* ledger, int slot, maua_stream_t stream) {
+    MAUA_REQUIRE(gy && bank && gx && x && ledger && slot >= 0 && slot < (1 << 28), MAUA_E_INVAL, "conv3x3_few_mfma_tv: bad args");
+    MAUA_REQUIRE(maua_conv_few_mfma_tv_supported(n, cin, h, w, cout, 1), MAUA_E_UNSUPPORTED, "conv3x3_few_mfma_tv: unsupported geometry");
+    MAUA_REQUIRE(tile >= 0 && tile <= 3, MAUA_E_INVAL, "conv3x3_few_mfma_tv: tile code 0 - 3");
+    FewMfmaArgs p{gy, (const unsigned char*)bank, gx, h, w, cin, 0, 0, 0, x, strength, ledger + (int64_t)slot * LEDGER_STRIDE};
+    return few_mfma_run(p, n, h, w, tile, true, (LEDGER_MAX / n) & ~7, (hipStream_t)stream);
+}
+
+}
diff --git a/maua-style_amd/csrc/conv_img.hip b/maua-style_amd/csrc/conv_img.hip
--- a/maua-style_amd/csrc/conv_img.hip
+++ b/maua-style_amd/csrc/conv_img.hip
@@ -61,7 +61,7 @@
     int64_t blocks;
 };
 
-template <bool GRAM>
+template <bool GRAM, bool NT>
 __global__ void __launch_bounds__(256, CI_OCC) conv_image_kernel(ImgArgs p) {
     const int lane = threadIdx.x & 63;
     const int nl = lane & 31, kg = lane >> 5;
@@ -189,7 +189,7 @@
                 const int cr = blk * 32 + (r & 3) + 8 * (r >> 2);
                 float o = acc[blk][r];
                 if (p.relu) o = o > 0.f ? o : 0.f;
-                __builtin_amdgcn_raw_buffer_store_b32(__builtin_bit_cast(unsigned, o), rs, voff, (int)(cr * out_plane * 4), 0);
+                __builtin_amdgcn_raw_buffer_store_b32(__builtin_bit_cast(unsigned, o), rs, voff, (int)(cr * out_plane * 4), NT ? 2 : 0);
             }
         if constexpr (GRAM) {
             ci_f32x16 xt[2];
@@ -325,7 +325,9 @@
     ImgArgs p{};
     const int rc = conv_image_fill(p, x, bank, y, n, cin, h, w, cout, pad, relu);
     if (rc) return rc;
-    hipLaunchKernelGGL(conv_image_kernel<false>, dim3(conv_image_grid(p.blocks), (unsigned)((cout + 63) / 64)), dim3(256), 0, (hipStream_t)stream, p);
+    const dim3 grid(conv_image_grid(p.blocks), (unsigned)((cout + 63) / 64));
+    if (tuning("image_nt", 0) != 0) hipLaunchKernelGGL((conv_image_kernel<false, true>), grid, dim3(256), 0, (hipStream_t)stream, p);
+    else hipLaunchKernelGGL((conv_image_kernel<false, false>), grid, dim3(256), 0, (hipStream_t)stream, p);
     return check_launch("conv_image_kernel");
 }
 
@@ -345,7 +347,9 @@
     const int rc = conv_image_fill(p, x, bank, y, 1, cin, h, w, 64, pad, 1);
     if (rc) return rc;
     p.gram_slabs = gram_slabs;
-    hipLaunchKernelGGL(conv_image_kernel<true>, dim3(conv_image_grid(p.blocks), 1), dim3(256), 0, (hipStream_t)stream, p);
+    const dim3 grid(conv_image_grid(p.blocks), 1);
+    if (tuning("image_nt", 0) != 0) hipLaunchKernelGGL((conv_image_kernel<true, true>), grid, dim3(256), 0, (hipStream_t)stream, p);
+    else hipLaunchKernelGGL((conv_image_kernel<true, false>), grid, dim3(256), 0, (hipStream_t)stream, p);
     return check_launch("conv_image_kernel");
 }
 
diff --git a/maua-style_amd/engine.py b/maua-style_amd/engine.py
--- a/maua-style_amd/engine.py
+++ b/maua-style_amd/engine.py
@@ -299,6 +299,16 @@
         else:
             gw = lw
         return lw, gw
+
+    def _tv_behind(self, s, shape):
+        if not plan.on("few_mfma_tv") or self.ledger is None or s.src != 0 or shape[0] != 1:
+            return None
+        for t in reversed(self.steps[:self.steps.index(s)]):
+            if t.kind == "tv":
+                return t
+            if not (t.kind == "content" and not self._active(t, shape)):
+                return None
+        return None
 
     def _active(self, s, shapes_src):
         m = s.mod
@@ -677,6 +687,8 @@
                                         self.slots[s.slot:s.slot + 1], workspace=self.ws, mask_grad_by_x=premask(s))
                     cur = s.src
             elif s.kind == "tv":
+                if id(s) in fused_done:
+                    continue
                 if self.ledger is not None:
                     hip.tv_fwd_bwd_ledger(a[0], g[0], s.mod.strength, cur == 0, self.ledger[0], s.slot)
                 else:
@@ -713,7 +725,13 @@
                     self._timed("conv_5x5_bwd", fl, nb, lambda: models_mod.conv5x5_mfma(
                         g[s.dst], s.mod, True, out=g[s.src], out_relu_mask=im, workspace=self.ws))
                 elif im is None and models_mod.conv_few_is_mfma(s.mod, *g[s.dst].shape[0:1], *g[s.dst].shape[2:]):
-                    self._timed("conv_other_bwd", fl, nb, lambda: models_mod.conv_few_mfma(g[s.dst], s.mod, g[s.src]))
+                    tv = self._tv_behind(s, a[0].shape) if not indep else None
+                    if tv is not None and hip.conv_few_mfma_tv_supported(*g[s.dst].shape[0:1], s.mod.in_channels, *g[s.dst].shape[2:], s.mod.out_channels, s.pad):
+                        self._timed("conv_other_bwd", fl, nb, lambda: models_mod.conv_few_mfma_tv(
+                            g[s.dst], s.mod, a[0], tv.mod.strength, self.ledger[0], tv.slot, g[s.src]))
+                        fused_done.add(id(tv))
+                    else:
+                        self._timed("conv_other_bwd", fl, nb, lambda: models_mod.conv_few_mfma(g[s.dst], s.mod, g[s.src]))
                 elif id(s) in self.strided_sites and im is None:
                     self._timed("conv_other_bwd", fl, nb, lambda: models_mod.conv_strided_bwd_as_3x3(
                         g[s.dst], s.mod, g[s.src], workspace=self.ws, sites=self.strided_sites[id(s)]))
diff --git a/maua-style_amd/hip.py b/maua-style_amd/hip.py
--- a/maua-style_amd/hip.py
+++ b/maua-style_amd/hip.py
@@ -70,6 +70,8 @@
     "maua_conv_pack_filters_few_mfma": (c_i, [c_p, c_p, c_i, c_i, c_p]),
     "maua_conv_few_mfma_supported": (c_i, [c_i, c_i, c_i, c_i, c_i, c_i]),
     "maua_conv3x3_few_mfma": (c_i, [c_p, c_p, c_p, c_i, c_i, c_i, c_i, c_i, c_i, c_p]),
+    "maua_conv_few_mfma_tv_supported": (c_i, [c_i, c_i, c_i, c_i, c_i, c_i]),
+    "maua_conv3x3_few_mfma_tv": (c_i, [c_p, c_p, c_p, c_p, c_i, c_i, c_i, c_i, c_i, c_i, c_f, c_p, c_i, c_p]),
     "maua_space_to_depth": (c_i, [c_p, c_p, c_i, c_i, c_i, c_i, c_i, c_i, c_i, c_p]),
     "maua_axpy": (c_i, [c_p, c_p, c_f, c_i64, c_p]),
     "maua_sum_small": (c_i, [c_p, c_i, c_p, c_p]),
@@ -864,6 +866,21 @@
     return out
 
 
+def conv_few_mfma_tv_supported(n, cin, h, w, cout, pad):
+    return bool(lib().maua_conv_few_mfma_tv_supported(int(n), int(cin), int(h), int(w), int(cout), int(pad)))
+
+
+def conv3x3_few_mfma_tv(gy, bank, x, strength, ledger, slot, out=None, tile=0):
+    n, cout, h, w = gy.shape
+    cin = x.shape[1]
+    assert tuple(x.shape) == (n, cin, h, w), (tuple(x.shape), tuple(gy.shape))
+    if out is None:
+        out = torch.empty(n, cin, h, w, device=gy.device, dtype=torch.float32)
+    _check(lib().maua_conv3x3_few_mfma_tv(_ptr(_f32(gy, "gy")), bank.data_ptr(), _ptr(out), _ptr(_f32(x, "x")), n, cin, h, w, cout, int(tile),
+                                          float(strength), ledger.data_ptr(), int(slot), _stream()), "maua_conv3x3_few_mfma_tv")
+    return out
+
+
 def space_to_depth(x, r, out):
     n, c, h, w = x.shape
     assert out.shape[0] == n and out.shape[1] == r * r * c
diff --git a/maua-style_amd/models.py b/maua-style_amd/models.py
--- a/maua-style_amd/models.py
+++ b/maua-style_amd/models.py
@@ -198,6 +198,11 @@
     return plan.on("few_mfma") and _x6_mode()[1] and k == 3 and stride == 1 and pad == 1 and hip.conv_few_mfma_supported(n, mod.in_channels, h, w, mod.out_channels, pad)
 
 
+def conv_few_mfma_tv(gy, mod, x, strength, ledger, slot, out):
+    _route("conv_few_mfma_tv", gy, mod.in_channels, 1, True, "4 / 8 x 62 px, bf16x6, TV loss in the epilogue")
+    return hip.conv3x3_few_mfma_tv(gy, mod.bank_few_mfma(), x, strength, ledger, slot, out=out)
+
+
 def conv_few_mfma(gy, mod, out):
     _route("conv_few_mfma", gy, mod.in_channels, 1, True, "4 / 8 x 62 px, bf16x6")
     return hip.conv3x3_few_mfma(gy, mod.bank_few_mfma(), mod.in_channels, out=out)
diff --git a/maua-style_amd/plan.py b/maua-style_amd/plan.py
--- a/maua-style_amd/plan.py
+++ b/maua-style_amd/plan.py
@@ -13,6 +13,7 @@
     "split_min_produced": ("16", "host", "a 3x3 stride-1 pass runs the split-precision kernels (64-channel tiles) when it PRODUCES at least this many channels, else the fp32-MFMA / direct kernels (VGG-19 / NIN: only the 64 -> 3 image gradient is below; the pruned VGG-16 has widths of 22 and 24)"),
     "x3w_min_pixels": ("4096", "host", "planes smaller than this run conv_x3.hip's 4-row tiles"),
     "few_mfma": ("1", "host", "backward-data of the image layer (64 -> 3 channels) on the matrix cores (conv_few_mfma.hip) instead of conv3x3_few_out's vector-ALU kernel"),
+    "few_mfma_tv": ("1", "host", "the TV loss that follows the image layer's backward pass rides in conv_few_mfma's epilogue: its gradient added to the value about to be stored, its loss as one ledger partial per workgroup (0: tv_kernel in a launch of its own)"),
     "strided_fwd_3x3": ("1", "host", "forward pass of a strided, unpadded layer (NIN's stem) as space to depth + a stride-1 3x3 convolution over sites (conv_x3w)"),
     "strided_bwd_3x3": ("1", "host", "backward-data of a strided, unpadded layer (NIN's 11x11 / 4 stem) as a stride-1 3x3 convolution over the output sites + depth to space"),
     "pool_codes": ("1", "host", "2x2 / 2 max pools keep one decision byte per window for the backward pass"),
@@ -47,6 +48,9 @@
     "x3p_groups": ("256", "lib", "conv_x3p: workgroups per launch (a multiple of 8)"),
     "x3p_min_fill": ("0.8", "lib", "conv_x3p_preferred: smallest list fill x plane cover"),
     "x3p_min_items": ("512", "lib", "conv_x3p_preferred: smallest number of work items (and a quarter of the smallest items x chunks)"),
+    "few_mfma_groups": ("0", "lib", "conv_few_mfma: at most this many workgroups per image, each walking several tiles of its XCD's band with the next tile's first loads in flight under the gather (0: a workgroup per tile)"),
+    "few_mfma_nt": ("0", "lib", "conv_few_mfma: the gradient map, read once, is loaded with the non-temporal hint"),
+    "image_nt": ("0", "lib", "conv_img: the activation map is stored with the non-temporal hint"),
     "x6_persist": ("0", "lib", "conv_x6: several tiles per workgroup (experiment)"),
     "gram_x3": ("1", "lib", "Gram partial products in fp16x3 (0: fp32 MFMA)"),
     "gram_bwd_x3": ("1", "lib", "Gram backward in fp16x3 (0: fp32 MFMA)"),
```

New measurement: 200.1. Within noise of the previous version (-0.2%).
